# abiswas-odu/Disco

Hardware: AMD Instinct MI355X
Metric: overlaps/sec (BuildGraph stage), 150 bp reads (higher is better)
Workload: dtype u64; 1 GPU; 50000000 x 150 bp synthetic reads, 30x of 50 x 5000000 bp uniform-random contigs, both strands, error-free, min-overlap 40 (k=39), transitive reduction on, seed 42; reads=50000000, read_len=150, min_overlap=40, parallelism=1 GPU, e_pre=903537181, e_out=45314794, n_contained=4685156, cap_bind_sites=0, asymmetric_pairs=0, probes=5550000000, kmer_hits=2220071992

## Files before the change

disco_amd/build.py:

```python
from __future__ import annotations

import os
import shutil
import subprocess

HERE = os.path.dirname(os.path.abspath(__file__))
ROOT = os.path.dirname(HERE)
LIB = os.path.join(HERE, "libdisco_hip.so")
BUILDG = os.path.join(HERE, "bin", "buildG")

HIP_SOURCES = [os.path.join(HERE, "csrc", "disco_hip.hip")]
HIP_DEPS = HIP_SOURCES + [os.path.join(HERE, "csrc", f) for f in sorted(f for f in os.listdir(os.path.join(HERE, "csrc")) if f.endswith(".h"))] + [
    os.path.join(ROOT, "include", "disco_hip.h"), os.path.join(ROOT, "include", "disco_hip_test.h")]
HOST_SOURCES = [os.path.join(HERE, "host", f) for f in ("buildg_main.cpp", "fastx.cpp", "writer.cpp", "parsimple.cpp")]


def _hipcc() -> str:
    for cand in (shutil.which("hipcc"), "/opt/rocm/bin/hipcc"):
        if cand and os.path.exists(cand):
            return cand
    raise RuntimeError("hipcc not found: the HIP extension cannot be built")


def _stale(target: str, deps) -> bool:
    if not os.path.exists(target):
        return True
    t = os.path.getmtime(target)
    return any(os.path.exists(d) and os.path.getmtime(d) > t for d in deps)


def vgpr_spills(remarks: str) -> dict:
    out, name = {}, None
    for line in remarks.splitlines():
        if "Function Name:" in line:
            name = line.split("Function Name:")[1].split("[")[0].strip()
        elif "VGPRs Spill:" in line and name:
            n = int(line.split("VGPRs Spill:")[1].split("[")[0])
            if n:
                out[name] = n
    return out


def build_lib(force: bool = False, verbose: bool = False) -> str:
    if force or _stale(LIB, HIP_DEPS):
        tmp = LIB + ".tmp"
        cmd = [_hipcc(), "--offload-arch=gfx950", "-O3", "-std=c++17", "-fPIC", "-shared", "-pthread", "-Rpass-analysis=kernel-resource-usage",
               "-o", tmp] + HIP_SOURCES + ["-L/opt/rocm/lib", "-lrccl", "-lrocprofiler-sdk-roctx", "-Wl,-rpath,/opt/rocm/lib"]
        if verbose:
            print(" ".join(cmd))
        r = subprocess.run(cmd, stdout=subprocess.PIPE, stderr=subprocess.PIPE, text=True)
        if r.returncode != 0:
            raise RuntimeError("hipcc failed:\n" + "\n".join(l for l in r.stderr.splitlines() if "-Rpass-analysis" not in l)[-4000:])
        spills = vgpr_spills(r.stderr)
        if spills and not os.environ.get("DISCO_ALLOW_SPILLS"):
            os.unlink(tmp)
            raise RuntimeError(f"kernels spill vector registers (cross-lane reads would return garbage): {spills}")
        os.replace(tmp, LIB)
    return LIB


def build_host(force: bool = False, verbose: bool = False) -> str:
    srcs = [s for s in HOST_SOURCES if os.path.exists(s)]
    if not srcs:
        return ""
    deps = srcs + [os.path.join(HERE, "host", f) for f in os.listdir(os.path.join(HERE, "host")) if f.endswith(".h")] + [LIB]
    if force or _stale(BUILDG, deps):
        os.makedirs(os.path.dirname(BUILDG), exist_ok=True)
        cmd = ["g++", "-O2", "-std=c++17", "-fopenmp", "-Wall", "-I", os.path.join(ROOT, "include"), "-o", BUILDG] + srcs + [
            "-L", HERE, "-ldisco_hip", "-lz", "-Wl,-rpath,$ORIGIN/..", "-Wl,-rpath," + HERE]
        if verbose:
            print(" ".join(cmd))
        subprocess.check_call(cmd)
    dump = os.path.join(HERE, "bin", "fastx_dump")
    dsrc = [os.path.join(HERE, "host", "fastx_dump.cpp"), os.path.join(HERE, "host", "fastx.cpp")]
    if force or _stale(dump, dsrc + [os.path.join(HERE, "host", "fastx.h")]):
        cmd = ["g++", "-O2", "-std=c++17", "-fopenmp", "-Wall", "-o", dump] + dsrc + ["-lz"]
        if verbose:
            print(" ".join(cmd))
        subprocess.check_call(cmd)
    ps = os.path.join(HERE, "bin", "parsimplify")
    psrc = [os.path.join(HERE, "host", f) for f in ("parsimplify_main.cpp", "parsimple.cpp", "fastx.cpp", "writer.cpp")]
    if force or _stale(ps, psrc + [os.path.join(HERE, "host", f) for f in ("parsimple.h", "writer.h", "fastx.h")]):
        cmd = ["g++", "-O2", "-std=c++17", "-fopenmp", "-Wall", "-I", os.path.join(ROOT, "include"), "-o", ps] + psrc + ["-lz"]
        if verbose:
            print(" ".join(cmd))
        subprocess.check_call(cmd)
    gen = os.path.join(HERE, "bin", "readgen")
    gsrc = [os.path.join(HERE, "host", "readgen_main.cpp"), os.path.join(HERE, "csrc", "readgen.h")]
    if force or _stale(gen, gsrc):
        cmd = ["g++", "-O2", "-std=c++17", "-Wall", "-o", gen, gsrc[0]]
        if verbose:
            print(" ".join(cmd))
        subprocess.check_call(cmd)
    chk = os.path.join(HERE, "bin", "inflate_check")
    csrc = [os.path.join(HERE, "host", "inflate_check.cpp"), os.path.join(HERE, "csrc", "disco_inflate.h")]
    if force or _stale(chk, csrc):
        cmd = ["g++", "-O2", "-std=c++17", "-Wall", "-o", chk, csrc[0]]
        if verbose:
            print(" ".join(cmd))
        subprocess.check_call(cmd)
    return BUILDG


def build_all(force: bool = False, verbose: bool = False):
    build_lib(force, verbose)
    build_host(force, verbose)


if __name__ == "__main__":
    build_all(force=True, verbose=True)
```

disco_amd/buildgraph.py:

```python
from __future__ import annotations

import ctypes as C
import os

import numpy as np

_HERE = os.path.dirname(os.path.abspath(__file__))
_LIBPATH = os.environ.get("DISCO_LIB") or os.path.join(_HERE, "libdisco_hip.so")
_lib = None


class DiscoError(RuntimeError):
    pass


class Params(C.Structure):
    _fields_ = [("min_overlap", C.c_uint32), ("max_edges_per_kmer", C.c_uint32), ("flags", C.c_uint32), ("max_substitutions", C.c_uint32)]


class GenSpecABI(C.Structure):
    _fields_ = [("seed", C.c_uint64), ("n_reads", C.c_uint64), ("contig_len", C.c_uint64), ("n_contigs", C.c_uint32),
                ("len_min", C.c_uint32), ("len_max", C.c_uint32), ("skew", C.c_uint32)]


CONTAINED_DTYPE = np.dtype([("contained", "<u8"), ("super", "<u8"), ("orient", "<u4"), ("len2", "<u4"), ("len1", "<u4"),
                            ("start", "<u4"), ("j", "<u4"), ("type", "<u4")])
EDGE_DTYPE = np.dtype([("src", "<u8"), ("dst", "<u8"), ("orient", "<u4"), ("offset", "<u4"), ("len_src", "<u4"), ("len_dst", "<u4")])
COUNTER_NAMES = ("n_reads", "probes", "kmer_hits", "n_contained", "raw_hits", "e_pre", "e_out", "cap_bind_sites",
                 "asymmetric_pairs", "big_rows", "index_buckets", "hbm_bytes")


class Counters(C.Structure):
    _fields_ = [(n, C.c_uint64) for n in COUNTER_NAMES]


_P = C.c_void_p
ABI = [
    ("disco_abi_version", C.c_int, []),
    ("disco_create", C.c_int, [C.c_int, C.POINTER(Params), C.POINTER(_P)]),
    ("disco_destroy", None, [_P]),
    ("disco_last_error", C.c_char_p, [_P]),
    ("disco_set_stream", C.c_int, [_P, _P]),
    ("disco_synchronize", C.c_int, [_P]),
    ("disco_pack_ascii", C.c_int, [C.c_char_p, C.c_uint32, _P]),
    ("disco_host_alloc", _P, [C.c_size_t]),
    ("disco_host_free", None, [_P]),
    ("disco_upload_reads", C.c_int, [_P, _P, C.c_uint32, _P, C.c_uint64]),
    ("disco_adopt_reads", C.c_int, [_P, _P, C.c_uint32, _P, C.c_uint64]),
    ("disco_generate_reads", C.c_int, [_P, C.POINTER(GenSpecABI)]),
    ("disco_substitute_bases", C.c_int, [_P, C.c_uint64, C.c_uint32]),
    ("disco_download_reads", C.c_int, [_P, _P, _P]),
    ("disco_stride_words", C.c_uint32, [_P]),
    ("disco_num_reads", C.c_uint64, [_P]),
    ("disco_long_rows", C.c_uint64, [_P]),
    ("disco_upload_reads_ragged", C.c_int, [_P, _P, _P, C.c_uint64]),
    ("disco_set_query_range", C.c_int, [_P, C.c_uint64, C.c_uint64]),
    ("disco_build_index", C.c_int, [_P]),
    ("disco_probe", C.c_int, [_P]),
    ("disco_mark_contained", C.c_int, [_P, C.POINTER(C.c_uint64)]),
    ("disco_build_edges", C.c_int, [_P, C.POINTER(C.c_uint64)]),
    ("disco_select_edges", C.c_int, [_P]),
    ("disco_symmetrize", C.c_int, [_P, C.c_int, C.POINTER(C.c_uint64)]),
    ("disco_merge_extras", C.c_int, [_P]),
    ("disco_transitive_reduce", C.c_int, [_P, C.POINTER(C.c_uint64)]),
    ("disco_transitive_mark", C.c_int, [_P]),
    ("disco_emit_edges", C.c_int, [_P, C.POINTER(C.c_uint64)]),
    ("disco_run_graph", C.c_int, [_P]),
    ("disco_adjacency_size", C.c_int, [_P, C.POINTER(C.c_uint64)]),
    ("disco_export_adjacency", C.c_int, [_P, _P, _P]),
    ("disco_import_adjacency", C.c_int, [_P, _P, _P, C.c_uint64]),
    ("disco_fetch_contained", C.c_int64, [_P, _P, C.c_uint64]),
    ("disco_fetch_contained_grouped", C.c_int64, [_P, _P, C.c_uint64]),
    ("disco_fetch_edges", C.c_int64, [_P, _P, C.c_uint64]),
    ("disco_fetch_edge_substitutions", C.c_int64, [_P, _P, C.c_uint64]),
    ("disco_get_counters", C.c_int, [_P, C.POINTER(Counters)]),
    ("disco_phase_ms", C.c_int, [_P, C.POINTER(C.c_float), C.c_int]),
    ("disco_memcpy_d2d", C.c_int, [_P, _P, _P, C.c_uint64]),
    ("disco_fetch_edge_files", C.c_int64, [_P, C.c_uint32, _P, C.c_uint64]),
    ("disco_partition_edges", C.c_int64, [_P, _P, C.c_uint64, C.c_uint64, C.c_uint32, _P]),
    ("disco_format_edges", C.c_int64, [_P, C.c_uint32, _P, _P, _P]),
    ("disco_fetch_edge_text", C.c_int, [_P, _P, C.c_uint64]),
    ("disco_write_edge_text", C.c_int, [_P, _P, C.c_uint32, C.c_uint32]),
    ("disco_start_contained_rows", C.c_int, [_P, C.c_int]),
    ("disco_contract_chains", C.c_int, [_P, C.c_uint32, C.POINTER(C.c_uint64), C.POINTER(C.c_uint64)]),
    ("disco_contract_chains_of", C.c_int, [_P, _P, C.c_uint64, C.c_uint32, C.POINTER(C.c_uint64), C.POINTER(C.c_uint64)]),
    ("disco_fetch_chains", C.c_int, [_P, _P, _P, _P]),
    ("disco_set_query_order", C.c_int, [_P, _P]),
    ("disco_get_query_order", C.c_int, [_P, C.POINTER(_P)]),
    ("disco_probe_run_words", C.c_int, [_P]),
    ("disco_measure_hbm", C.c_int, [_P, C.c_uint64, C.c_int, C.POINTER(C.c_double)]),
    ("disco_measure_gather", C.c_int, [_P, C.c_uint64, C.c_int, C.POINTER(C.c_double)]),
    ("disco_comm_unique_id", C.c_int, [_P, C.c_size_t]),
    ("disco_comm_init", C.c_int, [_P, _P, C.c_int, C.c_int]),
    ("disco_comm_init_local", C.c_int, [C.POINTER(_P), C.c_int]),
    ("disco_comm_rank", C.c_int, [_P]),
    ("disco_comm_world", C.c_int, [_P]),
    ("disco_comm_kind", C.c_char_p, [_P]),
    ("disco_dist_range", C.c_int, [_P, C.c_uint64, C.POINTER(C.c_uint64), C.POINTER(C.c_uint64)]),
    ("disco_dist_upload_reads", C.c_int, [_P, _P, C.c_uint32, _P, C.c_uint64]),
    ("disco_dist_generate_reads", C.c_int, [_P, C.POINTER(GenSpecABI)]),
    ("disco_dist_run_graph", C.c_int, [_P, C.c_uint32]),
    ("disco_dist_get_info", C.c_int, [_P, _P]),
    ("disco_ingest_fasta", C.c_int, [_P, C.POINTER(C.c_char_p), C.c_int, C.c_uint32, _P, _P]),
    ("disco_ingest_fetch", C.c_int, [_P, _P, _P]),
    ("disco_inflate_bgzf", C.c_int64, [_P, _P, C.c_uint64, _P, C.c_uint64]),
]

ABI_VERSION = 2
FLAG_TWO_PASS_VERIFY = 1
XCHG = ("reads", "index_records", "index_shards", "contain", "row_requests", "row_data", "push", "adjacency", "twins", "queries", "hits", "keys", "reads_dealt", "contain_keys")
UNIQUE_ID_BYTES = 128
DIST_GATHER_READS = 1
DIST_KEEP_INDEX_PARTITIONED = 2


CHAIN_EDGE_DTYPE = np.dtype([("a", "<u8"), ("b", "<u8"), ("offset", "<u8"), ("orient", "<u4"), ("n_links", "<u4"), ("first_link", "<u8")])
CHAIN_LINK_DTYPE = np.dtype([("to", "<u4"), ("offset", "<u4"), ("orient", "<u4")])


class IngestFile(C.Structure):
    _fields_ = [("first_index", C.c_uint64), ("last_index", C.c_uint64), ("good", C.c_uint64), ("bad", C.c_uint64)]


class IngestInfo(C.Structure):
    _fields_ = [("n_reads", C.c_uint64), ("total_records", C.c_uint64), ("too_long", C.c_uint64), ("stride_words", C.c_uint32), ("shortest", C.c_uint32),
                ("longest", C.c_uint32), ("read_s", C.c_float), ("device_s", C.c_float)]


class DistInfo(C.Structure):
    _fields_ = [("world", C.c_uint32), ("rank", C.c_uint32), ("n_reads", C.c_uint64), ("own_lo", C.c_uint64), ("own_hi", C.c_uint64),
                ("n_contained", C.c_uint64), ("e_pre", C.c_uint64), ("e_out", C.c_uint64), ("e_out_local", C.c_uint64),
                ("n_contained_local", C.c_uint64), ("cap_bind_sites", C.c_uint64), ("asymmetric_pairs", C.c_uint64),
                ("dropped_hits", C.c_uint64), ("probes", C.c_uint64), ("kmer_hits", C.c_uint64), ("regime", C.c_uint32),
                ("tr_rounds", C.c_uint32), ("tr_deferred", C.c_uint64), ("bytes_sent", C.c_uint64 * len(XCHG)),
                ("ms", C.c_float * len(XCHG)), ("ms_total", C.c_float), ("kernel_ms", C.c_float), ("comm_ops", C.c_uint32),
                ("host_syncs", C.c_uint32), ("device_allocs", C.c_uint32), ("device_frees", C.c_uint32), ("arena_bytes", C.c_uint64),
                ("arena_peak", C.c_uint64), ("hbm_peak", C.c_uint64), ("own_reads", C.c_uint64), ("placement", C.c_uint32), ("reserved_", C.c_uint32)]

PHASES = ("index", "probe_kernel", "verify", "contain", "select", "csr", "twin", "trmark", "emit", "order")


def lib_path() -> str:
    return _LIBPATH


def load():
    global _lib
    if _lib is None:
        if not os.path.exists(_LIBPATH):
            raise DiscoError(f"{_LIBPATH} is missing: build it with `python -m disco_amd.build` (hipcc, gfx950). "
                             "There is no CPU fallback.")
        L = C.CDLL(_LIBPATH)
        L.disco_abi_version.restype = C.c_int
        if L.disco_abi_version() != ABI_VERSION:
            raise DiscoError(f"{_LIBPATH} speaks ABI version {L.disco_abi_version()}, this mirror was written against {ABI_VERSION}: rebuild "
                             "(`python -m disco_amd.build`)")
        for name, res, args in ABI:
            fn = getattr(L, name)
            fn.restype = res
            fn.argtypes = args
        _lib = L
    return _lib


class BuildGraph:

    def __init__(self, min_overlap: int = 40, device: int = 0, max_edges_per_kmer: int = 4, flags: int = 0, max_substitutions: int = 0):
        self.L = load()
        self.min_overlap = min_overlap
        self._h = _P()
        p = Params(min_overlap, max_edges_per_kmer, flags, max_substitutions)
        rc = self.L.disco_create(device, C.byref(p), C.byref(self._h))
        if rc != 0:
            raise DiscoError(f"disco_create failed ({rc}): {self.L.disco_last_error(None).decode()}")

    def _chk(self, rc):
        if rc < 0:
            raise DiscoError(f"libdisco_hip error {rc}: {self.L.disco_last_error(self._h).decode()}")
        return rc

    def close(self):
        if self._h:
            self.L.disco_destroy(self._h)
            self._h = _P()

    def __del__(self):
        try:
            self.close()
        except Exception:
            pass

    def __enter__(self):
        return self

    def __exit__(self, *a):
        self.close()

    def set_stream(self, stream_ptr: int | None):
        self._chk(self.L.disco_set_stream(self._h, _P(stream_ptr) if stream_ptr else None))

    def synchronize(self):
        self._chk(self.L.disco_synchronize(self._h))

    def upload_reads(self, packed: np.ndarray, lens: np.ndarray):
        packed = np.ascontiguousarray(packed, dtype=np.uint64)
        lens = np.ascontiguousarray(lens, dtype=np.uint16)
        assert packed.ndim == 2 and packed.shape[0] == lens.shape[0]
        self._keep = (packed, lens)
        self._chk(self.L.disco_upload_reads(self._h, packed.ctypes.data, packed.shape[1], lens.ctypes.data, packed.shape[0]))

    def upload_reads_ragged(self, words: np.ndarray, lens: np.ndarray):
        words = np.ascontiguousarray(words, dtype=np.uint64)
        lens = np.ascontiguousarray(lens, dtype=np.uint16)
        assert words.ndim == 1 and len(words) == int(((lens.astype(np.int64) + 31) // 32).sum())
        self._chk(self.L.disco_upload_reads_ragged(self._h, words.ctypes.data, lens.ctypes.data, len(lens)))

    def upload_ascii(self, reads, ragged: bool = False):
        n = len(reads)
        lens = np.fromiter((len(r) for r in reads), dtype=np.uint16, count=n)
        if ragged:
            off = np.zeros(n + 1, dtype=np.int64)
            np.cumsum((lens.astype(np.int64) + 31) // 32, out=off[1:])
            words = np.zeros(max(int(off[-1]), 1), dtype=np.uint64)
            for i, r in enumerate(reads):
                b = r.encode()
                if self.L.disco_pack_ascii(b, len(b), words[off[i]:].ctypes.data) != 0:
                    raise DiscoError(f"read {i} contains a non-ACGT base")
            return self.upload_reads_ragged(words[:int(off[-1])], lens)
        stride = int((int(lens.max()) + 31) // 32) if n else 1
        packed = np.zeros((n, stride), dtype=np.uint64)
        for i, r in enumerate(reads):
            b = r.encode()
            if self.L.disco_pack_ascii(b, len(b), packed[i].ctypes.data) != 0:
                raise DiscoError(f"read {i} contains a non-ACGT base")
        self.upload_reads(packed, lens)

    def adopt_reads(self, d_packed_ptr: int, stride_words: int, d_len_ptr: int, n: int):
        self._chk(self.L.disco_adopt_reads(self._h, _P(d_packed_ptr), stride_words, _P(d_len_ptr), n))

    def generate_reads(self, spec):
        s = GenSpecABI(spec.seed, spec.n_reads, spec.contig_len, spec.n_contigs, spec.len_min, spec.len_max, int(spec.skew_word if hasattr(spec, "skew_word") else getattr(spec, "skew", 0)))
        self._chk(self.L.disco_generate_reads(self._h, C.byref(s)))

    def substitute_bases(self, seed: int, rate_ppm: int):
        self._chk(self.L.disco_substitute_bases(self._h, seed, rate_ppm))

    def download_reads(self):
        n, s = self.num_reads, self.stride_words
        packed = np.zeros((n, s), dtype=np.uint64)
        lens = np.zeros(n, dtype=np.uint16)
        self._chk(self.L.disco_download_reads(self._h, packed.ctypes.data, lens.ctypes.data))
        return packed, lens

    @property
    def num_reads(self) -> int:
        return int(self.L.disco_num_reads(self._h))

    @property
    def stride_words(self) -> int:
        return int(self.L.disco_stride_words(self._h))

    @property
    def long_rows(self) -> int:
        return int(self.L.disco_long_rows(self._h))

    def set_query_range(self, lo: int, hi: int):
        self._chk(self.L.disco_set_query_range(self._h, lo, hi))

    def build_index(self):
        self._chk(self.L.disco_build_index(self._h))

    def probe(self):
        self._chk(self.L.disco_probe(self._h))

    def mark_contained(self) -> int:
        n = C.c_uint64()
        self._chk(self.L.disco_mark_contained(self._h, C.byref(n)))
        return n.value

    def build_edges(self) -> int:
        n = C.c_uint64()
        self._chk(self.L.disco_build_edges(self._h, C.byref(n)))
        return n.value

    def select_edges(self):
        self._chk(self.L.disco_select_edges(self._h))

    def symmetrize(self, full: bool) -> int:
        n = C.c_uint64()
        self._chk(self.L.disco_symmetrize(self._h, 1 if full else 0, C.byref(n)))
        return n.value

    def merge_extras(self):
        self._chk(self.L.disco_merge_extras(self._h))

    def transitive_reduce(self) -> int:
        n = C.c_uint64()
        self._chk(self.L.disco_transitive_reduce(self._h, C.byref(n)))
        return n.value

    def transitive_mark(self):
        self._chk(self.L.disco_transitive_mark(self._h))

    def emit_edges(self) -> int:
        n = C.c_uint64()
        self._chk(self.L.disco_emit_edges(self._h, C.byref(n)))
        return n.value

    def run_graph(self):
        self._chk(self.L.disco_run_graph(self._h))

    def adjacency_size(self) -> int:
        n = C.c_uint64()
        self._chk(self.L.disco_adjacency_size(self._h, C.byref(n)))
        return n.value

    def export_adjacency(self, d_deg_ptr: int, d_entries_ptr: int):
        self._chk(self.L.disco_export_adjacency(self._h, _P(d_deg_ptr), _P(d_entries_ptr)))

    def import_adjacency(self, d_deg_all_ptr: int, d_entries_all_ptr: int, n_entries: int):
        self._chk(self.L.disco_import_adjacency(self._h, _P(d_deg_all_ptr), _P(d_entries_all_ptr), n_entries))

    def fetch_contained(self) -> np.ndarray:
        n = self._chk(self.L.disco_fetch_contained(self._h, None, 0))
        out = np.zeros(n, dtype=CONTAINED_DTYPE)
        if n:
            self._chk(self.L.disco_fetch_contained(self._h, out.ctypes.data, n))
        return out

    def fetch_contained_grouped(self):
        n = self._chk(self.L.disco_fetch_contained_grouped(self._h, None, 0))
        out = np.zeros(n, dtype=CONTAINED_DTYPE)
        if n:
            rc = self.L.disco_fetch_contained_grouped(self._h, out.ctypes.data, n)
            if rc == -6:
                return None
            self._chk(rc)
        return out

    def fetch_edges(self) -> np.ndarray:
        n = self._chk(self.L.disco_fetch_edges(self._h, None, 0))
        out = np.zeros(n, dtype=EDGE_DTYPE)
        if n:
            self._chk(self.L.disco_fetch_edges(self._h, out.ctypes.data, n))
        return out

    def format_edges(self, n_files: int = 1, edge_file=None, file_index=None):
        off = np.zeros(n_files + 1, dtype=np.uint64)
        ef = None if edge_file is None else np.ascontiguousarray(edge_file, dtype=np.uint16)
        fi = None if file_index is None else np.ascontiguousarray(file_index, dtype=np.uint64)
        nb = self._chk(self.L.disco_format_edges(self._h, n_files, None if ef is None else ef.ctypes.data, None if fi is None else fi.ctypes.data, off.ctypes.data))
        buf = np.empty(max(nb, 1), dtype=np.uint8)
        self._chk(self.L.disco_fetch_edge_text(self._h, buf.ctypes.data, nb))
        return buf[:nb].tobytes(), off

    def write_edge_text(self, fds, threads: int = 8):
        arr = (C.c_int * len(fds))(*fds)
        self._chk(self.L.disco_write_edge_text(self._h, arr, len(fds), threads))

    def start_contained_rows(self, grouped: bool = False):
        self._chk(self.L.disco_start_contained_rows(self._h, 1 if grouped else 0))

    def contract_chains(self, min_overlap_simplify: int = 0, edges=None):
        nc, nl = C.c_uint64(), C.c_uint64()
        if edges is None:
            self._chk(self.L.disco_contract_chains(self._h, min_overlap_simplify, C.byref(nc), C.byref(nl)))
            ne = int(self.L.disco_fetch_edges(self._h, None, 0))
        else:
            edges = np.ascontiguousarray(edges, dtype=EDGE_DTYPE)
            self._chk(self.L.disco_contract_chains_of(self._h, edges.ctypes.data, len(edges), min_overlap_simplify, C.byref(nc), C.byref(nl)))
            ne = len(edges)
        comp = np.zeros(nc.value, dtype=CHAIN_EDGE_DTYPE)
        links = np.zeros(nl.value, dtype=CHAIN_LINK_DTYPE)
        absorbed = np.zeros(ne, dtype=np.uint8)
        self._chk(self.L.disco_fetch_chains(self._h, comp.ctypes.data if len(comp) else None, links.ctypes.data if len(links) else None,
                                            absorbed.ctypes.data if ne else None))
        return comp, links, absorbed

    def fetch_edge_substitutions(self) -> np.ndarray:
        n = self._chk(self.L.disco_fetch_edge_substitutions(self._h, None, 0))
        out = np.zeros(n, dtype=np.uint16)
        if n:
            self._chk(self.L.disco_fetch_edge_substitutions(self._h, out.ctypes.data, n))
        return out

    def phase_ms(self) -> dict:
        a = (C.c_float * len(PHASES))()
        self._chk(self.L.disco_phase_ms(self._h, a, len(PHASES)))
        return {n: float(a[i]) for i, n in enumerate(PHASES)}

    def fetch_edge_files(self, n_files: int):
        n = int(self.L.disco_fetch_edges(self._h, None, 0))
        out = np.zeros(max(n, 1), dtype=np.uint16)
        self._chk(self.L.disco_fetch_edge_files(self._h, n_files, out.ctypes.data, n))
        return out[:n]

    def partition_edges(self, edges: np.ndarray, n_nodes: int, n_files: int):
        edges = np.ascontiguousarray(edges, dtype=EDGE_DTYPE)
        out = np.zeros(max(len(edges), 1), dtype=np.uint16)
        self._chk(self.L.disco_partition_edges(self._h, edges.ctypes.data, len(edges), n_nodes, n_files, out.ctypes.data))
        return out[:len(edges)]

    def get_query_order(self) -> int:
        out = _P()
        self._chk(self.L.disco_get_query_order(self._h, C.byref(out)))
        return out.value or 0

    def set_query_order(self, d_order_ptr: int):
        self._chk(self.L.disco_set_query_order(self._h, _P(d_order_ptr)))

    def probe_run_words(self) -> int:
        return int(self.L.disco_probe_run_words(self._h))

    def measure_hbm(self, nbytes: int = 4 << 30, reps: int = 5) -> float:
        out = C.c_double(0.0)
        self._chk(self.L.disco_measure_hbm(self._h, nbytes, reps, C.byref(out)))
        return out.value

    def measure_gather(self, nbytes: int = 3 << 30, reps: int = 3) -> float:
        out = C.c_double(0.0)
        self._chk(self.L.disco_measure_gather(self._h, nbytes, reps, C.byref(out)))
        return out.value

    def memcpy_d2d(self, dst_ptr: int, src_ptr: int, nbytes: int):
        self._chk(self.L.disco_memcpy_d2d(self._h, _P(dst_ptr), _P(src_ptr), nbytes))

    @staticmethod
    def comm_unique_id() -> bytes:
        buf = C.create_string_buffer(UNIQUE_ID_BYTES)
        rc = load().disco_comm_unique_id(buf, UNIQUE_ID_BYTES)
        if rc != 0:
            raise DiscoError(f"disco_comm_unique_id failed ({rc})")
        return buf.raw

    def comm_init(self, unique_id: bytes, world: int, rank: int):
        self._chk(self.L.disco_comm_init(self._h, C.c_char_p(unique_id), world, rank))

    @staticmethod
    def comm_init_local(graphs):
        arr = (_P * len(graphs))(*[g._h for g in graphs])
        rc = load().disco_comm_init_local(arr, len(graphs))
        if rc != 0:
            raise DiscoError(f"disco_comm_init_local failed ({rc})")

    @property
    def rank(self) -> int:
        return int(self.L.disco_comm_rank(self._h))

    @property
    def world(self) -> int:
        return int(self.L.disco_comm_world(self._h))

    @property
    def transport(self) -> str:
        return self.L.disco_comm_kind(self._h).decode()

    def dist_range(self, n_total: int):
        lo, hi = C.c_uint64(), C.c_uint64()
        self._chk(self.L.disco_dist_range(self._h, n_total, C.byref(lo), C.byref(hi)))
        return lo.value, hi.value

    def dist_upload_reads(self, packed_own: np.ndarray, lens_own: np.ndarray, n_total: int, stride_words: int | None = None):
        packed_own = np.ascontiguousarray(packed_own, dtype=np.uint64)
        lens_own = np.ascontiguousarray(lens_own, dtype=np.uint16)
        self._keep = (packed_own, lens_own)
        stride = int(stride_words if stride_words is not None else packed_own.shape[1])
        self._chk(self.L.disco_dist_upload_reads(self._h, packed_own.ctypes.data, stride, lens_own.ctypes.data, n_total))

    def dist_upload_ascii(self, reads):
        n = len(reads)
        lo, hi = self.dist_range(n)
        stride = int((max((len(r) for r in reads), default=1) + 31) // 32)
        packed = np.zeros((hi - lo, stride), dtype=np.uint64)
        lens = np.fromiter((len(r) for r in reads[lo:hi]), dtype=np.uint16, count=hi - lo)
        for i, r in enumerate(reads[lo:hi]):
            b = r.encode()
            if self.L.disco_pack_ascii(b, len(b), packed[i].ctypes.data) != 0:
                raise DiscoError(f"read {lo + i} contains a non-ACGT base")
        self.dist_upload_reads(packed, lens, n, stride)

    def dist_generate_reads(self, spec):
        s = GenSpecABI(spec.seed, spec.n_reads, spec.contig_len, spec.n_contigs, spec.len_min, spec.len_max, int(spec.skew_word if hasattr(spec, "skew_word") else getattr(spec, "skew", 0)))
        self._chk(self.L.disco_dist_generate_reads(self._h, C.byref(s)))

    def ingest_fasta(self, paths, threads: int = 16):
        arr = (C.c_char_p * len(paths))(*[os.fsencode(p) for p in paths])
        info, files = IngestInfo(), (IngestFile * len(paths))()
        rc = self.L.disco_ingest_fasta(self._h, arr, len(paths), threads, C.byref(info), files)
        if rc == -6:
            return None
        self._chk(rc)
        return ({n: getattr(info, n) for n, _ in IngestInfo._fields_}, [{n: getattr(f, n) for n, _ in IngestFile._fields_} for f in files])

    def inflate_bgzf(self, data: bytes):
        data = bytes(data)
        n = self.L.disco_inflate_bgzf(self._h, data, len(data), None, 0)
        if n == -6:
            return None
        out = C.create_string_buffer(max(self._chk(n), 1))
        n = self.L.disco_inflate_bgzf(self._h, data, len(data), out, n)
        if n == -6:
            return None
        return out.raw[:self._chk(n)]

    def last_error(self) -> str:
        return self.L.disco_last_error(self._h).decode()

    def ingest_fetch(self):
        n = self.num_reads
        ln, fi = np.zeros(n, dtype=np.uint16), np.zeros(n, dtype=np.uint64)
        self._chk(self.L.disco_ingest_fetch(self._h, ln.ctypes.data, fi.ctypes.data))
        return ln, fi

    def dist_run_graph(self, gather_reads: bool = True, partitioned_index: bool = False):
        self._chk(self.L.disco_dist_run_graph(self._h, (DIST_GATHER_READS if gather_reads else 0) | (DIST_KEEP_INDEX_PARTITIONED if partitioned_index else 0)))

    def dist_info(self) -> dict:
        d = DistInfo()
        self._chk(self.L.disco_dist_get_info(self._h, C.byref(d)))
        out = {n: getattr(d, n) for n, _ in DistInfo._fields_ if n not in ("bytes_sent", "ms")}
        out["bytes_sent"] = {x: int(d.bytes_sent[i]) for i, x in enumerate(XCHG)}
        out["ms"] = {x: float(d.ms[i]) for i, x in enumerate(XCHG)}
        return out

    def host_to_host_pass(self, passes: int = 2) -> dict:
        import time

        n, s = self.num_reads, self.stride_words
        p = self.L.disco_host_alloc(max(n * s * 8, 8))
        if not p:
            raise DiscoError("disco_host_alloc failed")
        q = None
        try:
            lens = np.zeros(n, dtype=np.uint16)
            self._chk(self.L.disco_download_reads(self._h, p, lens.ctypes.data))
            w = max(1, (int(lens.max()) + 31) // 32) if n else 1
            src, sw = p, s
            if w < s:
                q = self.L.disco_host_alloc(max(n * w * 8, 8))
                if not q:
                    raise DiscoError("disco_host_alloc failed")
                full = np.ctypeslib.as_array(C.cast(p, C.POINTER(C.c_uint64)), shape=(n, s))
                np.ctypeslib.as_array(C.cast(q, C.POINTER(C.c_uint64)), shape=(n, w))[:] = full[:, :w]
                src, sw = q, w
            rows = edges = None
            out, first = {}, None
            for ip in range(max(1, passes)):
                t0 = time.perf_counter()
                self._chk(self.L.disco_upload_reads(self._h, src, sw, lens.ctypes.data, n))
                t1 = time.perf_counter()
                self.run_graph()
                self.synchronize()
                t2 = time.perf_counter()
                nc = self._chk(self.L.disco_fetch_contained(self._h, None, 0))
                ne = self._chk(self.L.disco_fetch_edges(self._h, None, 0))
                if rows is None or len(rows) < nc or len(edges) < ne:
                    rows = np.zeros(max(nc, 1), dtype=CONTAINED_DTYPE)
                    edges = np.zeros(max(ne, 1), dtype=EDGE_DTYPE)
                t3 = time.perf_counter()
                if nc:
                    self._chk(self.L.disco_fetch_contained(self._h, rows.ctypes.data, nc))
                t4 = time.perf_counter()
                if ne:
                    self._chk(self.L.disco_fetch_edges(self._h, edges.ctypes.data, ne))
                t5 = time.perf_counter()
# ... 17 lines not shown
```

disco_amd/csrc/disco_hip.hip:

```cpp
#include <hip/hip_runtime.h>
#include <rocprofiler-sdk-roctx/roctx.h>

#include <algorithm>
#include <atomic>
#include <chrono>
#include <cstdarg>
#include <cstdio>
#include <cstdlib>
#include <cstring>
#include <fcntl.h>
#include <sys/mman.h>
#include <sys/stat.h>
#include <unistd.h>
#include <string>
#include <memory>
#include <thread>
#include <map>
#include <mutex>
#include <vector>

#include "../../include/disco_hip.h"
#include "../../include/disco_hip_test.h"
#include "disco_kernels.h"
#include "disco_dist.h"

#define DROP_LIST_CAP (1u << 20)
#include "disco_chains.h"
#include "disco_text.h"
#include "disco_ingest.h"
#include "disco_bgzf.h"
#include "read_filter_tables.h"
#include "disco_comm.h"

static_assert(sizeof(disco_genspec) == sizeof(disco_genspec_abi), "genspec ABI mismatch");

static thread_local std::string g_create_error;

using HClock = std::chrono::steady_clock;
static float ms_since(HClock::time_point t0) { return std::chrono::duration<float, std::milli>(HClock::now() - t0).count(); }

#define DISCO_PH_INDEX2 DISCO_PH_COUNT
#define DISCO_PH_SLOTS (DISCO_PH_COUNT + 1)

struct RoctxRange {
    explicit RoctxRange(const char *name) { (void)roctxRangePushA(name); }
    ~RoctxRange() { (void)roctxRangePop(); }
    RoctxRange(const RoctxRange &) = delete;
    RoctxRange &operator=(const RoctxRange &) = delete;
};
#define DISCO_TRACE(name) RoctxRange roctx_range_(name)

template <typename F>
static void parallel_for(u64 n, F f)
{
    unsigned nt = std::thread::hardware_concurrency();
    if (const char *e = getenv("DISCO_HOST_THREADS")) nt = (unsigned)atoi(e);
    nt = std::max(1u, std::min(nt, 16u));
    if (n < (1u << 16) || nt == 1) {
        f((u64)0, n);
        return;
    }
    std::vector<std::thread> th;
    for (unsigned t = 0; t < nt; t++) th.emplace_back([=]() { f(n * t / nt, n * (t + 1) / nt); });
    for (auto &x : th) x.join();
}


struct PassCounters {
    u32 dev_allocs = 0, dev_frees = 0, host_syncs = 0, comm_ops = 0;
};
static thread_local PassCounters tl_pass;
static inline hipError_t counted_stream_sync(hipStream_t s)
{
    tl_pass.host_syncs++;
    return hipStreamSynchronize(s);
}
static inline hipError_t counted_event_sync(hipEvent_t e)
{
    tl_pass.host_syncs++;
    return hipEventSynchronize(e);
}
#define hipStreamSynchronize(s) counted_stream_sync(s)
#define hipEventSynchronize(e) counted_event_sync(e)

struct DevArena {
    char *base = nullptr;
    size_t size = 0, used = 0, peak = 0;
    std::map<size_t, size_t> free_at;
    bool owns(const void *p) const { return base && (const char *)p >= base && (const char *)p < base + size; }
    void *alloc(size_t bytes)
    {
        bytes = (bytes + 255) & ~(size_t)255;
        for (auto it = free_at.begin(); it != free_at.end(); ++it)
            if (it->second >= bytes) {
                const size_t off = it->first, len = it->second;
                free_at.erase(it);
                if (len > bytes) free_at[off + bytes] = len - bytes;
                live[off] = bytes;
                used += bytes;
                peak = std::max(peak, used);
                return base + off;
            }
        return nullptr;
    }
    void release(void *p)
    {
        const size_t off = (size_t)((char *)p - base);
        auto lv = live.find(off);
        if (lv == live.end()) return;
        size_t start = off, end = off + lv->second;
        used -= lv->second;
        live.erase(lv);
        auto nx = free_at.lower_bound(off);
        if (nx != free_at.end() && nx->first == end) {
            end += nx->second;
            nx = free_at.erase(nx);
        }
        if (nx != free_at.begin()) {
            auto pv = std::prev(nx);
            if (pv->first + pv->second == start) {
                start = pv->first;
                free_at.erase(pv);
            }
        }
        free_at[start] = end - start;
    }
    std::map<size_t, size_t> live;
};

template <typename T>
struct DevBuf {
    T *p = nullptr;
    u64 cap = 0;
    operator T *() const { return p; }
};

struct disco_ctx {
    int device = 0;
    disco_params prm{};
    DevArena arena;
    int k = 0;
    hipStream_t own_stream = nullptr;
    hipStream_t stream = nullptr;
    int n_cu = 256;
    std::string err;
    size_t hbm_bytes = 0, hbm_peak = 0;

    u64 n = 0;
    int S = 0;
    u64 *d_reads = nullptr;
    u16 *d_len = nullptr;
    DevBuf<u64> reads_own;
    DevBuf<u16> len_own;
    bool reads_owned = false;
    std::vector<uint16_t> h_len;
    bool h_len_ok = false;
    std::mutex h_len_mu;
    u64 q_lo = 0, q_hi = 0;
    bool two_class = false;
    bool dist_two_class = false;
    u64 job_n_long = 0;
    u32 job_short_max = 0;
    int S_ext = 0;
    u64 n_long = 0;
    DevBuf<u64> d_full;
    DevBuf<u32> d_ovf, d_long_ids;
    u32 max_len_all = 0;
    int tailb = 0;
    DevBuf<u32> d_lpos, d_n_list;
    DevBuf<uint2> d_linfo;
    DevBuf<ulonglong2> d_lmeta;

    u64 T = 0;
    int bshift = 0;
    DevBuf<u32> d_bkt;
    DevBuf<u64> d_ent;
    DevBuf<ulonglong2> d_rec;
    bool binned_index = false;
    DevBuf<ulonglong2> d_rec2;
    DevBuf<u32> d_binx;

    DevBuf<u64> d_tile;
    u64 *d_total = nullptr;

    u64 *d_ctr = nullptr;
    u64 *d_wq = nullptr;
    u64 h_ctr[CTR_COUNT] = {0};

    DevBuf<u64> d_best;
    DevBuf<u64> d_hits;
    u64 hits_used = 0;
    u64 *d_bump = nullptr;
    DevBuf<u64> d_row_start;
    DevBuf<u32> d_row_cnt;
    DevBuf<u64> d_big_list;
    DevBuf<u32> d_big_cnt;
    u32 *d_n_big = nullptr;
    DevBuf<u32> d_runs;
    u64 runs_lo = 0, runs_n = 0;
    int runs_lpr = 0;
    DevBuf<u64> d_slow_list;
    u32 *d_n_slow = nullptr;
    u64 big_rows = 0, slow_rows = 0;
    const u64 *d_order = nullptr;
    const u64 *d_order_used = nullptr;
    bool order_external = false;
    DevBuf<u32> d_ocnt, d_okey, d_oslot;
    DevBuf<u64> d_order_own;
    bool order_counted = false;
    bool es_big_counted = false, tr_big_counted = false;
    bool contained_count_pending = false;
    bool order_ready = false;
    hipStream_t aux_stream = nullptr;
    hipEvent_t ev_crows = nullptr;
    DevBuf<u32> d_cpos, d_crow_id;
    DevBuf<u64> d_crow_key;
    DevBuf<u64> d_tile2;
    u64 *d_total2 = nullptr;
    void *h_crows = nullptr;
    DevBuf<u32> d_crow_len;
    u64 crows_hcap = 0, crows_n = 0;
    bool crows_pending = false;
    bool crows_in_ring = false;
    DevBuf<u32> d_cgrp_cur, d_cgrp_id;
    DevBuf<u64> d_cgrp_key, d_cgrp_big;
    u64 h_cgrp_big = 0;
    bool cgrp_pending = false;
    DevBuf<u32> d_fetch_src;
    DevBuf<u64> d_fetch_ent;
    DevBuf<u32> d_rec_of_read;
    std::vector<u64> ingest_id_base, ingest_rec_base;
    u64 ingest_n = 0;
    void *h_ring = nullptr;
    std::vector<u64> text_off;
    DevBuf<u8> d_ingest;
    std::thread hits_prealloc;
    DevBuf<u64> prealloc;
    size_t ring_half = 0;
    hipEvent_t ev_ring[2] = {nullptr, nullptr};
    hipStream_t copy_stream = nullptr;
    hipEvent_t ev_copied[3] = {nullptr, nullptr, nullptr}, ev_unpacked[3] = {nullptr, nullptr, nullptr};
    bool index_counted = false;
    u64 order_counted_lo = 0, order_counted_hi = 0;
    int order_counted_bits = 0;
    DevBuf<u32> d_asked;
    u64 order_q_lo = 0, order_q_hi = 0;
    DevBuf<ulonglong2> d_meta_ord;
    u64 dropped_local = 0;
    ProbeRare h_probe_rare;
    DevBuf<ProbeRare> d_probe_rare;
    u32 max_len = 0, min_len = 0;
    bool two_pass_last = false;
    bool contained_done = false;

    DevBuf<u8> d_contained;
    DevBuf<u64> d_cbits;
    DevBuf<u64> d_dropbits;
    DevBuf<u64> d_drop_node, d_drop_key;
    u64 n_drop_items = 0;
    u64 drop_lo = 0, drop_hi = 0;
    u64 n_contained = 0;

    DevBuf<u64> d_adj_ref;
    u64 *d_adj = nullptr;
    DevBuf<u64> d_adj_own;
    DevBuf<u64> d_adj_spare;
    DevBuf<u64> d_start_tmp;
    u64 adj_total = 0;
    bool flags_pending = false;
    bool adj_imported = false;
    u64 adj_span = 0;
    bool half_complete = false;
    DevBuf<u32> d_extra_cnt;
    DevBuf<u64> d_extra_node, d_extra_key;
    u32 *d_n_extra = nullptr;
    u32 n_extra = 0;
    u64 asym_local = 0;
    u64 dropped = 0;

    DevBuf<u64> d_half;
    DevBuf<u32> d_hcnt;
    bool use_half = false;
    DevBuf<u64> d_wide;
    DevBuf<u32> d_n_wide;
    u32 n_wide = 0;
    DevBuf<u8> d_out_valid;
    DevBuf<u64> d_out_pos;
    u64 *h_stage = nullptr;
    hipEvent_t ev_stage[2] = {nullptr, nullptr};
    DevBuf<ChainEdgeOut> d_ch_comp;
    DevBuf<ChainLinkOut> d_ch_links;
    DevBuf<u8> d_ch_dead;
    u64 ch_comp_n = 0, ch_links_n = 0, ch_edges_n = 0;
    bool ch_ready = false;
    DevBuf<char> d_text;
    u64 text_bytes = 0;
    DevBuf<u64> d_out_src, d_out_ent;
    u64 out_used = 0;
    u64 n_out = 0;

    hipEvent_t ev0[DISCO_PH_SLOTS] = {nullptr}, ev1[DISCO_PH_SLOTS] = {nullptr};
    bool ev_pending[DISCO_PH_SLOTS] = {false};
    float ph_ms[DISCO_PH_SLOTS] = {0};

    int phase = 0;

    DiscoComm *comm = nullptr;
    DiscoComm *comm_bulk = nullptr;
    hipStream_t bulk_stream = nullptr;
    hipEvent_t ev_bulk = nullptr;
    bool wait_bulk_before_verify = false;
    u64 per = 0;
    u64 n_alloc = 0;
    bool part_index = false;
    u64 part_blo = 0, part_bhi = 0, part_nrec = 0;
    DevBuf<u64> d_pq_start;
    bool dist_reads = false;
    bool dist_active = false;
    DevBuf<u64> d_route;
    DevBuf<ulonglong2> d_x16a, d_x16b;
    DevBuf<u32> d_req_flat, d_req_s, d_req_r;
    DevBuf<u32> d_rdeg_s, d_rdeg_r, d_rdata_s;
    DevBuf<u64> d_rpos;
    DevBuf<u32> d_nadj32_own;
    u64 nadj_used = 0;
    DevBuf<u32> d_deg_tmp;
    DevBuf<u64> d_list_n;
    DevBuf<u64> d_dense;
    ulonglong2 *d_push_r = nullptr;
    u64 n_push_r = 0;
    bool loci = false;
    bool runs_by_pos = false;
    DevBuf<u8> d_otab;
    DevBuf<u32> d_own_ids;
    u64 n_own = 0;
    u64 home_lo = 0, home_hi = 0;
    u64 home_probes = 0;
    DevBuf<u64> d_cb_all;
    hipEvent_t ev_keys = nullptr, ev_keys_go = nullptr;
    bool keys_pending = false;
    disco_dist_info dinfo{};
    bool time_exchanges = false;
    unsigned dist_passes = 0;
};

static int fail(disco_ctx *c, int code, const char *fmt, ...)
{
    char buf[512];
    va_list ap;
    va_start(ap, fmt);
    vsnprintf(buf, sizeof buf, fmt, ap);
    va_end(ap);
    if (c) c->err = buf;
    else g_create_error = buf;
    return code;
}

#define HIPCHK(c, call)                                                                                          \
    do {                                                                                                         \
        hipError_t e_ = (call);                                                                                  \
        if (e_ != hipSuccess) return fail((c), e_ == hipErrorOutOfMemory ? DISCO_E_NOMEM : DISCO_E_HIP, "%s failed: %s (%s:%d)", #call, hipGetErrorString(e_), __FILE__, __LINE__); \
    } while (0)
// ... 231 lines not shown

template <typename InT, typename OutT>
static int scan_exclusive_on(disco_ctx *c, hipStream_t st, DevBuf<u64> &tile, u64 *total, const InT *in, u64 n, OutT *out, bool write_total, u64 *total_host)
{
    u64 nt = (n + SCAN_TILE - 1) / SCAN_TILE;
    if (nt == 0) nt = 1;
    CHK(ensure(c, tile, nt));
    hipLaunchKernelGGL((scan_tile_sums_kernel<InT>), dim3((unsigned)nt), dim3(SCAN_BLOCK), 0, st, in, n, tile.p);
    hipLaunchKernelGGL(scan_sums_kernel, dim3(1), dim3(1024), 0, st, tile.p, nt, total);
    hipLaunchKernelGGL((scan_apply_kernel<InT, OutT>), dim3((unsigned)nt), dim3(SCAN_BLOCK), 0, st, in, n, tile.p, out);
    if (write_total) hipLaunchKernelGGL((scan_write_total_kernel<OutT>), dim3(1), dim3(1), 0, st, total, out + n);
    HIPCHK(c, hipGetLastError());
    if (total_host) {
        HIPCHK(c, hipMemcpyAsync(total_host, total, sizeof(u64), hipMemcpyDeviceToHost, st));
        HIPCHK(c, hipStreamSynchronize(st));
    }
    return DISCO_OK;
}

template <typename InT, typename OutT>
static int scan_exclusive(disco_ctx *c, const InT *in, u64 n, OutT *out, bool write_total, u64 *total_host)
{
    return scan_exclusive_on<InT, OutT>(c, c->stream, c->d_tile, c->d_total, in, n, out, write_total, total_host);
}

static void free_graph_state(disco_ctx *c)
{
    if (c->keys_pending) {
        c->keys_pending = false;
        if (c->ev_keys) (void)hipEventSynchronize(c->ev_keys);
    }
    release(c, c->d_bkt);
    release(c, c->d_ent);
    release(c, c->d_rec);
    release(c, c->d_rec2);
    release(c, c->d_binx);
    release(c, c->d_best);
    release(c, c->d_hits);
    release(c, c->d_row_start);
    release(c, c->d_row_cnt);
    release(c, c->d_big_list);
    release(c, c->d_big_cnt);
    release(c, c->d_slow_list);
    release(c, c->d_runs);
    c->runs_n = 0;
    c->runs_lpr = 0;
    release(c, c->d_contained);
    release(c, c->d_cbits);
    release(c, c->d_dropbits);
    release(c, c->d_drop_node);
    release(c, c->d_drop_key);
    release(c, c->d_adj_ref);
    release(c, c->d_adj_own);
    release(c, c->d_adj_spare);
    release(c, c->d_start_tmp);
    release(c, c->d_ocnt);
    release(c, c->d_okey);
    release(c, c->d_meta_ord);
    release(c, c->d_asked);
    release(c, c->d_oslot);
    release(c, c->d_order_own);
    c->d_order_used = nullptr;
    c->d_adj = nullptr;
    release(c, c->d_extra_cnt);
    release(c, c->d_extra_node);
    release(c, c->d_extra_key);
    release(c, c->d_half);
    release(c, c->d_hcnt);
    release(c, c->d_wide);
    release(c, c->d_n_wide);
    c->adj_total = 0;
    release(c, c->d_out_valid);
    release(c, c->d_ch_comp);
    release(c, c->d_ch_links);
    release(c, c->d_ch_dead);
    release(c, c->d_text);
    c->text_bytes = 0;
    c->ch_ready = false;
    release(c, c->d_out_pos);
    release(c, c->d_out_src);
    release(c, c->d_out_ent);
    c->n_out = c->out_used = 0;
    c->flags_pending = false;
    c->adj_imported = false;
    c->T = 0;
    release(c, c->d_x16a);
    release(c, c->d_x16b);
    release(c, c->d_req_flat);
    release(c, c->d_req_s);
    release(c, c->d_req_r);
    release(c, c->d_rdeg_s);
    release(c, c->d_rdeg_r);
    release(c, c->d_rdata_s);
    release(c, c->d_rpos);
    release(c, c->d_nadj32_own);
    release(c, c->d_deg_tmp);
    release(c, c->d_dense);
    release(c, c->d_pq_start);
    c->nadj_used = 0;
    c->d_push_r = nullptr;
    c->n_push_r = 0;
    release(c, c->d_cb_all);
    release(c, c->d_otab);
    release(c, c->d_own_ids);
    c->n_own = 0;
    c->loci = c->runs_by_pos = false;
}

static void free_long_class(disco_ctx *c)
{
    release(c, c->d_full);
    release(c, c->d_ovf);
    release(c, c->d_long_ids);
    release(c, c->d_lpos);
    release(c, c->d_lmeta);
    release(c, c->d_linfo);
    release(c, c->d_n_list);
    c->two_class = false;
    c->n_long = 0;
    c->S_ext = 0;
    c->tailb = 0;
}

static void free_reads(disco_ctx *c)
{
    release(c, c->reads_own);
    release(c, c->len_own);
    free_long_class(c);
    c->d_reads = nullptr;
    c->d_len = nullptr;
    c->reads_owned = false;
    c->h_len.clear();
    c->n = 0;
}

static int alloc_reads(disco_ctx *c, u64 words, u64 n_len)
{
    CHK(ensure(c, c->reads_own, words));
    c->d_reads = c->reads_own;
    CHK(ensure(c, c->len_own, n_len));
    c->d_len = c->len_own;
    return DISCO_OK;
}

static u32 extra_cap(const disco_ctx *c) { return (u32)std::min<u64>(std::min(c->d_extra_node.cap, c->d_extra_key.cap), 0xFFFFFFFFull); }

static int grow_big_lists(disco_ctx *c, u64 need) { return ensure_group(c, need, need, c->d_big_list, c->d_big_cnt); }

static bool own_order_wanted(const disco_ctx *c, u64 nq, int *bits)
{
    const u64 order_min = getenv("DISCO_ORDER_MIN_READS") ? (u64)atoll(getenv("DISCO_ORDER_MIN_READS")) : 4096;
    int b = 16;
    while (b < 27 && (1ull << b) < nq) ++b;
    *bits = b;
    return !c->order_external && !getenv("DISCO_NO_ORDER") && nq >= order_min && nq > 0;
}

struct IndexCountPlan {
    u64 lo = 0, hi = 0;
    int lpr = 0, nf = 0;
    u32 *ocnt = nullptr, *oslot = nullptr;
    u32 oshift = 0;
    const u64 *list = nullptr;
};

static bool runs_nf_built(int nf, int m) { return (nf == 7 || nf == 12 || nf == 17 || nf == 22 || nf == 27) && m == RUNS_M; }

static int runs_lpr_for(const disco_ctx *c, int nf, u32 max_len, u64 nloc)
{
    int lpr = 0;
    const int m = view(c).m;
    const bool nf_built = runs_nf_built(nf, m);
    const bool nf_generic = nf >= 2 && nf <= 64 && m > 16 && m <= 31 && !getenv("DISCO_NO_GENERIC_RUNS");
    if ((nf_built || nf_generic) && max_len > (u32)c->k && !getenv("DISCO_NO_RUNS")) {
        const u32 maxwin = max_len - (u32)c->k;
        const u32 expect = 2u * maxwin / (u32)(nf + 1);
        lpr = maxwin <= 256 ? (maxwin <= 128 && expect <= 20 ? 16 : (expect <= 44 ? 32 : 0)) : 0;
        const double max_gb = getenv("DISCO_RUNS_MAX_GB") ? atof(getenv("DISCO_RUNS_MAX_GB")) : 16.0;
        if ((double)nloc * lpr * 4.0 > max_gb * 1e9) lpr = 0;
    }
    return lpr;
}

static bool two_class_ok(const disco_ctx *c, int S, u64 n, u64 n_long, u32 short_max, bool will_own = false)
{
    if (((c->comm || c->dist_reads) && !c->dist_two_class) || !(c->reads_owned || will_own) || c->prm.max_substitutions || getenv("DISCO_NO_TWO_CLASS")) return false;
    if (S <= VERIFY_SW || n_long == 0 || n_long * (u64)env_int("DISCO_TWO_CLASS_ONE_IN", 5) > n || n + n_long >= (1ull << 31)) return false;
    return runs_lpr_for(c, c->k - view(c).m + 1, short_max, n) != 0;
}

static int two_class_alloc(disco_ctx *c, u64 n_long, int Sx, u32 short_max);

static int index_count_plan(disco_ctx *c, const DiscoView &v, u64 lo, u64 hi, IndexCountPlan *pl, const u64 *list = nullptr)
{
    const u64 nloc = hi - lo;
    *pl = IndexCountPlan();
    pl->lo = lo;
    pl->hi = hi;
    pl->list = list;
    if (!list) c->order_counted = c->order_ready = false;
    int obits = 0;
    if (!list && lo == c->q_lo && hi == c->q_hi && own_order_wanted(c, nloc, &obits) && !getenv("DISCO_NO_ORDER_FUSE")) {
        const u64 order_buckets = 1ull << obits;
        CHK(ensure(c, c->d_ocnt, order_buckets + 1));
        CHK(ensure(c, c->d_oslot, nloc));
        HIPCHK(c, hipMemsetAsync(c->d_ocnt, 0, (order_buckets + 1) * sizeof(u32), c->stream));
        pl->ocnt = c->d_ocnt;
        pl->oslot = c->d_oslot;
        pl->oshift = 32u - (u32)obits;
        c->order_counted = true;
        c->order_counted_lo = lo;
        c->order_counted_hi = hi;
        c->order_counted_bits = obits;
    }
    c->runs_lpr = 0;
    c->runs_n = 0;
    c->runs_by_pos = false;
    const int nf = v.k - v.m + 1;
    const int lpr = c->S == VERIFY_SW ? runs_lpr_for(c, nf, c->max_len, nloc) : 0;
    if (lpr && nloc) {
        CHK(ensure(c, c->d_runs, nloc * (u64)lpr));
        c->runs_lpr = lpr;
        c->runs_lo = lo;
        c->runs_n = nloc;
        c->runs_by_pos = list != nullptr;
        pl->lpr = lpr;
        pl->nf = nf;
    }
    return DISCO_OK;
}

typedef void (*IndexRunsFn)(DiscoView, u32 *, ulonglong2 *, u32 *, u64, u64, u32 *, u32 *, u32 *, u32, const u64 *);
typedef void (*IndexCountFn)(DiscoView, u32 *, ulonglong2 *, u32 *, u64, u64, u32 *, u32 *, u32, const u64 *);
struct IndexCountKernel {
    IndexRunsFn runs = nullptr;
    IndexCountFn plain = nullptr;
};
template <bool COUNT, int NF, int NFMAX, bool LONGK>
static IndexCountKernel index_runs_pick(int lpr)
{
    IndexCountKernel k;
    k.runs = lpr == 16 ? index_runs_kernel<COUNT, NF, 1, NFMAX, LONGK> : index_runs_kernel<COUNT, NF, 2, NFMAX, LONGK>;
    return k;
}
template <bool COUNT>
static IndexCountKernel index_count_pick(int nf, int m, int lpr, bool longk, bool long_class)
{
    if (long_class || !lpr) {
        IndexCountKernel k;
        if (long_class) k.plain = longk ? index_count_kernel<COUNT, true, true> : index_count_kernel<COUNT, false, true>;
        else k.plain = longk ? index_count_kernel<COUNT, true> : index_count_kernel<COUNT>;
        return k;
    }
    if (runs_nf_built(nf, m)) switch (nf) {
        case 7: return index_runs_pick<COUNT, 7, 7, false>(lpr);
        case 12: return index_runs_pick<COUNT, 12, 12, false>(lpr);
        case 17: return index_runs_pick<COUNT, 17, 17, false>(lpr);
        case 22: return index_runs_pick<COUNT, 22, 22, false>(lpr);
        default: return index_runs_pick<COUNT, 27, 27, false>(lpr);
        }
    if (longk) return nf <= 48 ? index_runs_pick<COUNT, 0, 48, true>(lpr) : index_runs_pick<COUNT, 0, 64, true>(lpr);
    if (nf <= 8) return index_runs_pick<COUNT, 0, 8, false>(lpr);
    if (nf <= 12) return index_runs_pick<COUNT, 0, 12, false>(lpr);
    if (nf <= 16) return index_runs_pick<COUNT, 0, 16, false>(lpr);
    if (nf <= 24) return index_runs_pick<COUNT, 0, 24, false>(lpr);
    if (nf <= 32) return index_runs_pick<COUNT, 0, 32, false>(lpr);
    if (nf <= 48) return index_runs_pick<COUNT, 0, 48, false>(lpr);
    return index_runs_pick<COUNT, 0, 64, false>(lpr);
}
static IndexCountKernel index_count_pick(bool count, int nf, int m, int lpr, bool longk, bool long_class)
{
    return count ? index_count_pick<true>(nf, m, lpr, longk, long_class) : index_count_pick<false>(nf, m, lpr, longk, long_class);
}

static int index_count_chunk(disco_ctx *c, const DiscoView &v, const IndexCountPlan &pl, bool count, ulonglong2 *rec_base, u64 a, u64 b)
{
    if (b <= a) return DISCO_OK;
    const dim3 grid((unsigned)((b - a + 255) / 256));
    ulonglong2 *rec = rec_base + 2 * (a - pl.lo);
    u32 *oslot = pl.oslot ? pl.oslot + (a - pl.lo) : nullptr;
    u32 *okey = pl.list ? nullptr : c->d_okey.p;
    const IndexCountKernel k = index_count_pick(count, pl.nf, v.m, pl.lpr, c->k > 64, false);
    if (k.runs) hipLaunchKernelGGL(k.runs, grid, dim3(256), 0, c->stream, v, c->d_bkt, rec, okey, a, b, c->d_runs + (a - pl.lo) * (u64)pl.lpr, pl.ocnt, oslot, pl.oshift, pl.list);
    else hipLaunchKernelGGL(k.plain, grid, dim3(256), 0, c->stream, v, c->d_bkt, rec, okey, a, b, pl.ocnt, oslot, pl.oshift, pl.list);
    HIPCHK(c, hipGetLastError());
    return DISCO_OK;
}

static int index_count_long(disco_ctx *c, const DiscoView &v, const IndexCountPlan &pl, bool count, ulonglong2 *rec, u32 *oslot, u64 x_lo, u64 x_hi)
{
    const dim3 g((unsigned)((x_hi - x_lo + 255) / 256));
    hipLaunchKernelGGL(index_count_pick(count, 0, v.m, 0, c->k > 64, true).plain, g, dim3(256), 0, c->stream, v, c->d_bkt, rec, c->d_okey, x_lo, x_hi, pl.ocnt, oslot, pl.oshift,
                       (const u64 *)nullptr);
    HIPCHK(c, hipGetLastError());
    return DISCO_OK;
}

static bool binned_index_wanted(disco_ctx *c, int logT)
{
    if (getenv("DISCO_NO_BINNED_INDEX") || 2 * c->n >= 0xFFFF0000ull) return false;
    if (logT > BINX_SPAN_BITS && ensure(c, c->d_rec2, 2 * c->n) != DISCO_OK) {
        (void)hipGetLastError();
        c->err.clear();
        return false;
    }
    return true;
}

static int size_bucket_table(disco_ctx *c)
{
    u64 T = 1024;
    int logT = 10;
    double tscale = 2.0;
    if (const char *e = getenv("DISCO_BUCKET_SCALE")) tscale = atof(e);
    while ((double)T < tscale * (double)c->n && logT < 32) {
        T <<= 1;
        logT++;
    }
    c->T = T;
    c->bshift = 64 - logT;
    return logT;
}

static int index_begin(disco_ctx *c)
{
    const int logT = size_bucket_table(c);
    const u64 T = c->T;
    CHK(ensure(c, c->d_bkt, T + 1));
    CHK(ensure(c, c->d_ent, 2 * c->n));
    CHK(ensure(c, c->d_rec, 2 * c->n));
    CHK(ensure(c, c->d_okey, c->n));
    c->adj_imported = false;
    c->binned_index = binned_index_wanted(c, logT);
    if (!c->binned_index) HIPCHK(c, hipMemsetAsync(c->d_bkt, 0, (T + 1) * sizeof(u32), c->stream));
    return DISCO_OK;
}

struct BinxPlan {
    int span = 0, levels = 0, bits[3] = {0, 0, 0};
};
static BinxPlan binx_plan(int logT)
{
    BinxPlan b;
    b.span = std::min(logT, BINX_SPAN_BITS);
    const int prefix = logT - b.span;
    b.levels = (prefix + BINX_MAX_BITS - 1) / BINX_MAX_BITS;
    for (int l = 0; l < b.levels; l++) b.bits[l] = prefix / b.levels + (l < prefix % b.levels ? 1 : 0);
    return b;
}

static int binned_build_index(disco_ctx *c)
{
    const int logT = 64 - c->bshift;
    const BinxPlan bp = binx_plan(logT);
    const u32 total = (u32)(2 * c->n);
    const u32 n_part = 1u << (logT - bp.span);
    const u32 tiles = (total + BINX_TILE - 1u) / BINX_TILE;
    u64 hist_len = 1;
    for (int l = 0, done = 0; l < bp.levels; done += bp.bits[l], l++) hist_len = std::max<u64>(hist_len, ((u64)tiles + (1ull << done)) * (1ull << bp.bits[l]) + 1);
    const u64 tab = ((u64)n_part + 1 + 63) & ~63ull;
    CHK(ensure(c, c->d_binx, 4 * tab + hist_len));
    u32 *seg[2] = {c->d_binx.p, c->d_binx.p + tab}, *tb[2] = {c->d_binx.p + 2 * tab, c->d_binx.p + 3 * tab}, *hist = c->d_binx.p + 4 * tab;
    if (getenv("DISCO_VERBOSE"))
        fprintf(stderr, "[disco] binned index build: 2^%d buckets, %u partitions of 2^%d, %d level(s) of %d / %d / %d bits\n", logT, n_part, bp.span, bp.levels, bp.bits[0], bp.bits[1], bp.bits[2]);
    ulonglong2 *src = c->d_rec, *dst = c->d_rec2;
    u32 pseg = 1, pnb = 1;
    int cur = 0, done = 0;
    for (int l = 0; l < bp.levels; l++) {
        const u32 nseg = 1u << done, nb = 1u << bp.bits[l], shift = (u32)(logT - done - bp.bits[l]);
        const u32 grid = tiles + nseg;
        const u64 hlen = (u64)grid * nb + 1;
        hipLaunchKernelGGL(binx_segs_kernel, dim3(1), dim3(1024), 0, c->stream, l ? (const u32 *)hist : (const u32 *)nullptr, (const u32 *)tb[cur ^ 1], pseg, pnb, total, seg[cur], tb[cur]);
        HIPCHK(c, hipMemsetAsync(hist, 0, hlen * sizeof(u32), c->stream));
        hipLaunchKernelGGL(binx_hist_kernel, dim3(grid), dim3(BINX_BLOCK), 0, c->stream, (const ulonglong2 *)src, (const u32 *)seg[cur], (const u32 *)tb[cur], nseg, shift, nb, hist);
        CHK((scan_exclusive<u32, u32>(c, hist, hlen, hist, false, nullptr)));
        hipLaunchKernelGGL(binx_scatter_kernel, dim3(grid), dim3(BINX_BLOCK), 0, c->stream, (const ulonglong2 *)src, dst, (const u32 *)seg[cur], (const u32 *)tb[cur], nseg, shift, nb,
                           (const u32 *)hist);
        HIPCHK(c, hipGetLastError());
        std::swap(src, dst);
        pseg = nseg;
        pnb = nb;
        done += bp.bits[l];
        cur ^= 1;
    }
    hipLaunchKernelGGL(binx_segs_kernel, dim3(1), dim3(1024), 0, c->stream, bp.levels ? (const u32 *)hist : (const u32 *)nullptr, (const u32 *)tb[cur ^ 1], pseg, pnb, total, seg[cur],
                       (u32 *)nullptr);
    hipLaunchKernelGGL(binx_build_kernel, dim3(n_part), dim3(BINX_BUILD_BLOCK), 0, c->stream, (const ulonglong2 *)src, (const u32 *)seg[cur], (u32)bp.span, total, c->T, c->d_bkt.p, c->d_ent.p);
    HIPCHK(c, hipGetLastError());
    return DISCO_OK;
}

static int start_contained_rows(disco_ctx *c, bool grouped)
{
    const u64 nc = c->n_contained;
    if (c->crows_pending && c->crows_n == nc && (!grouped || c->cgrp_pending)) return DISCO_OK;
    const bool have_rows = c->crows_pending && c->crows_n == nc;
    if (!have_rows) c->crows_pending = c->cgrp_pending = false;
    const u64 max_rows = getenv("DISCO_EAGER_ROWS_MAX") ? (u64)atoll(getenv("DISCO_EAGER_ROWS_MAX")) : (16ull << 20);
    if (c->comm || nc == 0 || nc > max_rows || c->n >= (1ull << 31)) return DISCO_OK;
    if (!c->aux_stream) {
        HIPCHK(c, hipStreamCreateWithFlags(&c->aux_stream, hipStreamNonBlocking));
        HIPCHK(c, hipEventCreateWithFlags(&c->ev_crows, hipEventDisableTiming));
        HIPCHK(c, hipMalloc((void **)&c->d_total2, sizeof(u64)));
    }
    CHK(ensure(c, c->d_cpos, c->n + 1));
    CHK(ensure_group(c, nc, nc + nc / 4 + 1024, c->d_crow_id, c->d_crow_key, c->d_crow_len));
    if (nc > c->crows_hcap && c->h_ring && !c->crows_in_ring && (u64)c->ring_half * 2 >= (nc + 1024) * 32) {
        if (c->h_crows) (void)hipHostFree(c->h_crows);
        c->h_crows = c->h_ring;
        c->crows_hcap = (u64)c->ring_half * 2 / 32;
        c->crows_in_ring = true;
    }
    if (nc > c->crows_hcap) {
        if (c->h_crows && !c->crows_in_ring) (void)hipHostFree(c->h_crows);
        c->crows_in_ring = false;
        c->h_crows = nullptr;
        c->crows_hcap = 0;
        const u64 want = nc + nc / 4 + 1024;
        if (hipHostMalloc(&c->h_crows, want * 32) != hipSuccess) {
            c->h_crows = nullptr;
            (void)hipGetLastError();
            return DISCO_OK;
        }
        c->crows_hcap = want;
    }
    if (!have_rows) {
    CHK((scan_exclusive_on<u8, u32>(c, c->aux_stream, c->d_tile2, c->d_total2, c->d_contained, c->n, c->d_cpos, false, nullptr)));
    hipLaunchKernelGGL(contain_rows32_kernel, dim3(flat_grid(c, c->n)), dim3(256), 0, c->aux_stream, c->d_best, c->d_contained, c->d_cpos, c->n, c->d_crow_id, c->d_crow_key);
    HIPCHK(c, hipGetLastError());
    u64 *hkey = (u64 *)c->h_crows;
    u32 *hid = (u32 *)(hkey + c->crows_hcap), *hln = hid + c->crows_hcap;
    hipLaunchKernelGGL(crow_lens_kernel, dim3(flat_grid(c, nc)), dim3(256), 0, c->aux_stream, (const u32 *)c->d_crow_id, (const u64 *)c->d_crow_key, nc, (const u16 *)c->d_len, c->d_crow_len);
    HIPCHK(c, hipGetLastError());
    HIPCHK(c, hipMemcpyAsync(hkey, c->d_crow_key, nc * 8, hipMemcpyDeviceToHost, c->aux_stream));
    HIPCHK(c, hipMemcpyAsync(hid, c->d_crow_id, nc * 4, hipMemcpyDeviceToHost, c->aux_stream));
    HIPCHK(c, hipMemcpyAsync(hln, c->d_crow_len, nc * 4, hipMemcpyDeviceToHost, c->aux_stream));
    HIPCHK(c, hipEventRecord(c->ev_crows, c->aux_stream));
    c->crows_n = nc;
    c->crows_pending = true;
    }
    if (grouped && !c->cgrp_pending) {
        CHK(ensure(c, c->d_cgrp_cur, c->n + 1));
        CHK(ensure_group(c, nc, nc + nc / 4 + 1024, c->d_cgrp_id, c->d_cgrp_key));
        CHK(ensure(c, c->d_cgrp_big, 1));
        HIPCHK(c, hipMemsetAsync(c->d_cpos, 0, (c->n + 1) * sizeof(u32), c->aux_stream));
        HIPCHK(c, hipMemsetAsync(c->d_cgrp_big, 0, sizeof(u64), c->aux_stream));
        hipLaunchKernelGGL(crow_count_kernel, dim3(flat_grid(c, nc)), dim3(256), 0, c->aux_stream, (const u64 *)c->d_crow_key, nc, c->d_cpos);
        CHK((scan_exclusive_on<u32, u32>(c, c->aux_stream, c->d_tile2, c->d_total2, c->d_cpos, c->n + 1, c->d_cgrp_cur, false, nullptr)));
        hipLaunchKernelGGL(crow_place_kernel, dim3(flat_grid(c, nc)), dim3(256), 0, c->aux_stream, (const u32 *)c->d_crow_id, (const u64 *)c->d_crow_key, nc, c->d_cgrp_cur, c->d_cgrp_id,
                           c->d_cgrp_key);
        hipLaunchKernelGGL(crow_sort_groups_kernel, dim3(flat_grid(c, nc)), dim3(256), 0, c->aux_stream, c->d_cgrp_id, c->d_cgrp_key, nc, c->d_cgrp_big);
        HIPCHK(c, hipGetLastError());
        u64 *gkey = (u64 *)((char *)c->h_crows + c->crows_hcap * 16);
        u32 *gid = (u32 *)(gkey + c->crows_hcap), *gln = gid + c->crows_hcap;
        hipLaunchKernelGGL(crow_lens_kernel, dim3(flat_grid(c, nc)), dim3(256), 0, c->aux_stream, (const u32 *)c->d_cgrp_id, (const u64 *)c->d_cgrp_key, nc, (const u16 *)c->d_len, c->d_crow_len);
        HIPCHK(c, hipMemcpyAsync(gkey, c->d_cgrp_key, nc * 8, hipMemcpyDeviceToHost, c->aux_stream));
        HIPCHK(c, hipMemcpyAsync(gid, c->d_cgrp_id, nc * 4, hipMemcpyDeviceToHost, c->aux_stream));
        HIPCHK(c, hipMemcpyAsync(gln, c->d_crow_len, nc * 4, hipMemcpyDeviceToHost, c->aux_stream));
        HIPCHK(c, hipMemcpyAsync(&c->h_cgrp_big, c->d_cgrp_big, sizeof(u64), hipMemcpyDeviceToHost, c->aux_stream));
        c->cgrp_pending = true;
    }
    return DISCO_OK;
}

static int settle_contained_rows(disco_ctx *c)
{
    if (c->crows_pending) HIPCHK(c, hipStreamSynchronize(c->aux_stream));
    c->crows_pending = false;
    c->cgrp_pending = false;
    return DISCO_OK;
}

static int ring_back_from_rows(disco_ctx *c)
{
    if (!c->crows_in_ring) return DISCO_OK;
    if (c->crows_pending && c->aux_stream) HIPCHK(c, hipStreamSynchronize(c->aux_stream));
    c->crows_pending = c->cgrp_pending = false;
    c->h_crows = nullptr;
    c->crows_hcap = 0;
    c->crows_in_ring = false;
    return DISCO_OK;
}

static void settle_hits_prealloc(disco_ctx *c)
{
    if (!c->hits_prealloc.joinable()) return;
    c->hits_prealloc.join();
    if (c->prealloc) {
        if (c->prealloc.cap > c->d_hits.cap) {
            release(c, c->d_hits);
            adopt(c, c->d_hits, c->prealloc);
        } else
            (void)hipFree(c->prealloc.p);
        c->prealloc = DevBuf<u64>();
    }
}


typedef void (*ProbeFn)(ProbeArgs);
typedef void (*ProbeRunsFn)(ProbeArgs, const u32 *, u64);
struct ProbeKernel {
    ProbeRunsFn runs = nullptr;
    ProbeFn plain = nullptr;
};
template <int PMODE>
static ProbeFn probe_mode_pick(bool ldsrow, bool row17, bool longk, bool long_class)
{
    if constexpr (PMODE != 0) {
        if (long_class) return longk ? probe_kernel<PMODE, false, false, true, true> : row17 ? probe_kernel<PMODE, false, true, false, true> : probe_kernel<PMODE, false, false, false, true>;
    }
    if constexpr (PMODE != 2) {
        if (!ldsrow) return longk ? probe_kernel<PMODE, false, false, true> : row17 ? probe_kernel<PMODE, false, true> : probe_kernel<PMODE, false, false>;
    }
    return longk ? probe_kernel<PMODE, true, false, true> : row17 ? probe_kernel<PMODE, true, true> : probe_kernel<PMODE, true, false>;
}
static ProbeKernel probe_pick(const disco_ctx *c, int mode, bool use_runs)
{
    const bool ldsrow = c->S <= PROBE_ACAP;
    const bool row17 = c->k - view(c).m == 16 && !getenv("DISCO_NO_ROW17");
    const bool longk = c->k > 64;
    const bool long_class = c->two_class && c->S_ext > PROBE_ACAP;
    ProbeKernel k;
    if (mode == 0 && use_runs) k.runs = c->runs_lpr == 16 ? probe_runs_kernel<16> : probe_runs_kernel<32>;
    else if (mode == 0) k.plain = probe_mode_pick<0>(ldsrow, row17, longk, long_class);
    else if (mode == 1) k.plain = probe_mode_pick<1>(ldsrow, row17, longk, long_class);
    else k.plain = probe_mode_pick<2>(ldsrow, row17, longk, long_class);
    return k;
}

typedef void (*VerifyFn)(VerifyArgs);
template <bool INEXACT>
static VerifyFn verify_rows_pick(int S, bool short_rows)
{
    if (S == VERIFY_SW) return short_rows ? verify_kernel<5, 0, INEXACT> : verify_kernel<8, 0, INEXACT>;
    return S == 16 ? verify_kernel<16, 0, INEXACT> : S == 24 ? verify_kernel<24, 0, INEXACT> : S == 32 ? verify_kernel<32, 0, INEXACT> : verify_kernel<0, 0, INEXACT>;
}
template <int MODE>
static VerifyFn verify_pass_pick(bool flat, bool short_rows)
{
    if (flat) return short_rows ? verify_flat_kernel<5, MODE> : verify_flat_kernel<8, MODE>;
// ... 1132 lines not shown
    if (s->len_min == 0 || s->len_max < s->len_min || longest > 32767 || s->n_contigs == 0 || s->contig_len < longest)
        return fail(c, DISCO_E_ARG, "disco_generate_reads: bad spec");
    HIPCHK(c, hipSetDevice(c->device));
    uint32_t stride = (((longest + 31) / 32) + 7u) & ~7u;
    bool kept = false;
    CHK(set_reads_common(c, s->n_reads, stride, &kept));
    if (!kept) CHK(alloc_reads(c, c->n * (u64)stride, c->n));
    c->reads_owned = true;
    disco_genspec g;
    memcpy(&g, s, sizeof g);
    if (c->n) hipLaunchKernelGGL(generate_reads_kernel, dim3(flat_grid(c, c->n * stride)), dim3(256), 0, c->stream, g, c->d_reads, c->d_len, (int)stride, (u64)0, c->n);
    HIPCHK(c, hipGetLastError());
    return validate_reads(c);
}

int disco_substitute_bases(disco_ctx *c, uint64_t seed, uint32_t rate_ppm)
{
    if (!c) return DISCO_E_ARG;
    if (c->phase != 1) return fail(c, DISCO_E_STATE, "disco_substitute_bases: call after the reads are set and before disco_build_index");
    if (rate_ppm > 1000000) return fail(c, DISCO_E_ARG, "disco_substitute_bases: rate above 10^6 ppm");
    if (c->two_class)
        return fail(c, DISCO_E_UNSUPPORTED, "disco_substitute_bases: the table has two classes of rows (reads of more than 256 bases next to short ones); substitute "
                                            "into generated reads, or set DISCO_NO_TWO_CLASS=1");
    HIPCHK(c, hipSetDevice(c->device));
    const u64 lo = c->comm ? c->q_lo : 0, hi = c->comm ? c->q_hi : c->n;
    if (hi > lo && rate_ppm)
        hipLaunchKernelGGL(substitute_bases_kernel, dim3(flat_grid(c, (hi - lo) * (u64)c->S)), dim3(256), 0, c->stream, (u64)seed, rate_ppm, c->d_reads, c->d_len, c->S, lo, hi);
    c->index_counted = c->order_counted = c->order_ready = false;
    HIPCHK(c, hipGetLastError());
    return DISCO_OK;
}

int disco_download_reads(disco_ctx *c, uint64_t *packed, uint16_t *len)
{
    if (!c || c->phase < 1) return c ? fail(c, DISCO_E_STATE, "no reads") : DISCO_E_ARG;
    HIPCHK(c, hipSetDevice(c->device));
    DevBuf<u64> joined;
    if (packed && c->n && c->two_class) {
        CHK(ensure(c, joined, c->n * (u64)c->S_ext));
        hipLaunchKernelGGL(class_join_kernel, dim3(flat_grid(c, c->n * (u64)c->S_ext)), dim3(256), 0, c->stream, (const u64 *)c->d_reads, (const u64 *)c->d_full, c->S_ext,
                           (const u16 *)c->d_len, (const u32 *)c->d_ovf, c->n, joined);
        (void)hipMemcpyAsync(packed, joined, c->n * (u64)c->S_ext * 8, hipMemcpyDeviceToHost, c->stream);
    } else if (packed && c->n)
        HIPCHK(c, hipMemcpyAsync(packed, c->d_reads, c->n * (u64)c->S * 8, hipMemcpyDeviceToHost, c->stream));
    if (len && c->n) (void)hipMemcpyAsync(len, c->d_len, c->n * 2, hipMemcpyDeviceToHost, c->stream);
    const hipError_t e = hipStreamSynchronize(c->stream);
    release(c, joined);
    if (e != hipSuccess) return fail(c, DISCO_E_HIP, "disco_download_reads: %s", hipGetErrorString(e));
    return DISCO_OK;
}

uint32_t disco_stride_words(const disco_ctx *c) { return c ? (uint32_t)(c->two_class ? c->S_ext : c->S) : 0; }
uint64_t disco_num_reads(const disco_ctx *c) { return c ? c->n : 0; }
uint64_t disco_long_rows(const disco_ctx *c) { return c && c->two_class ? c->n_long : 0; }

int disco_set_query_range(disco_ctx *c, uint64_t lo, uint64_t hi)
{
    if (!c) return DISCO_E_ARG;
    if (c->phase < 1 || c->phase > 2) return fail(c, DISCO_E_STATE, "disco_set_query_range: call after the reads are set and before disco_probe");
    if (lo > hi || hi > c->n) return fail(c, DISCO_E_ARG, "query range [%llu,%llu) outside [0,%llu)", (unsigned long long)lo, (unsigned long long)hi, (unsigned long long)c->n);
    c->q_lo = lo;
    c->q_hi = hi;
    return DISCO_OK;
}

static int two_class_alloc(disco_ctx *c, u64 n_long, int Sx, u32 short_max)
{
    c->n_long = n_long;
    c->S_ext = Sx;
    int rc = DISCO_OK;
    rc = ensure(c, c->d_ovf, c->n_alloc);
    if (rc == DISCO_OK) rc = ensure(c, c->d_full, n_long * (u64)Sx);
    if (rc == DISCO_OK) rc = ensure(c, c->d_long_ids, n_long);
    if (rc == DISCO_OK) rc = ensure(c, c->d_lpos, n_long);
    if (rc == DISCO_OK) rc = ensure(c, c->d_lmeta, n_long);
    if (rc == DISCO_OK) rc = ensure(c, c->d_linfo, n_long);
    if (rc == DISCO_OK) rc = ensure(c, c->d_n_list, 1);
    if (rc != DISCO_OK) {
        free_long_class(c);
        return rc;
    }
    c->S = VERIFY_SW;
    c->tailb = short_max <= 160 ? 160 : 256;
    c->two_class = true;
    if (getenv("DISCO_VERBOSE"))
        fprintf(stderr, "[disco] two classes of rows: %llu of %llu reads are longer than 256 bases, the others up to %u: 64-byte rows + %d-word rows for those\n",
                (unsigned long long)n_long, (unsigned long long)c->n, short_max, Sx);
    return DISCO_OK;
}

static int two_class_convert(disco_ctx *c)
{
    if (c->two_class || !c->n || c->max_len <= (u32)DISCO_SHORT_MAX || !two_class_ok(c, c->S, c->n, 1, (u32)c->k + 1)) return DISCO_OK;
    const int Sx = c->S;
    DevBuf<u32> ovf;
    CHK(ensure(c, ovf, c->n_alloc));
    CHK(zero_counter(c, CTR_SHORT_MAX));
    hipLaunchKernelGGL(class_flag_kernel, dim3(flat_grid(c, c->n)), dim3(256), 0, c->stream, c->d_len, c->n, ovf.p, c->d_ctr);
    u64 n_long = 0;
    CHK((scan_exclusive<u32, u32>(c, ovf, c->n, ovf, false, &n_long)));
    CHK(read_counters(c));
    const u32 short_max = (u32)c->h_ctr[CTR_SHORT_MAX];
    if (!two_class_ok(c, Sx, c->n, n_long, short_max)) {
        release(c, ovf);
        return DISCO_OK;
    }
    DevBuf<u64> rows8;
    c->d_ovf = ovf;
    int rca = ensure(c, rows8, (c->n + n_long) * 8);
    if (rca == DISCO_OK) rca = two_class_alloc(c, n_long, Sx, short_max);
    if (rca != DISCO_OK) {
        release(c, rows8);
        free_long_class(c);
        return rca;
    }
    hipLaunchKernelGGL(class_split_kernel, dim3(flat_grid(c, c->n * 8)), dim3(256), 0, c->stream, (const u64 *)c->reads_own, Sx, (const u16 *)c->d_len, (const u32 *)ovf, c->n, c->tailb,
                       rows8.p, c->d_full, c->d_long_ids);
    HIPCHK(c, hipGetLastError());
    HIPCHK(c, hipStreamSynchronize(c->stream));
    release(c, c->reads_own);
    c->reads_own = rows8;
    c->d_reads = c->reads_own;
    c->max_len_all = c->max_len;
    c->max_len = short_max;
    return DISCO_OK;
}

int disco_build_index(disco_ctx *c)
{
    DISCO_TRACE("disco_build_index");
    if (!c) return DISCO_E_ARG;
    if (c->phase < 1) return fail(c, DISCO_E_STATE, "disco_build_index: no reads");
    HIPCHK(c, hipSetDevice(c->device));
    ph_begin(c, DISCO_PH_INDEX);
    if (c->index_counted) {
        c->index_counted = false;
    } else {
        CHK(two_class_convert(c));
        CHK(index_begin(c));
        const DiscoView v = view(c);
        IndexCountPlan pl;
        CHK(index_count_plan(c, v, 0, c->n, &pl));
        CHK(index_count_chunk(c, v, pl, !c->binned_index, c->d_rec, 0, c->n));
        if (c->two_class) CHK(index_count_long(c, v, pl, !c->binned_index, c->d_rec, pl.oslot, 0, c->n_long));
    }
    const bool binned = c->binned_index;
    if (!binned) CHK((scan_exclusive<u32, u32>(c, c->d_bkt, c->T + 1, c->d_bkt, false, nullptr)));
    c->order_ready = false;
    if (c->order_counted && c->order_counted_lo == 0 && c->order_counted_hi == c->n && !c->two_class && !getenv("DISCO_NO_ORDERED_FILL")) {
        const u64 order_buckets = 1ull << c->order_counted_bits;
        CHK(ensure(c, c->d_order_own, c->n));
        ph_end(c, DISCO_PH_INDEX);
        ph_begin(c, DISCO_PH_ORDER);
        CHK((scan_exclusive<u32, u32>(c, c->d_ocnt, order_buckets + 1, c->d_ocnt, false, nullptr)));
        hipLaunchKernelGGL(order_scatter_kernel, dim3(flat_grid(c, c->n)), dim3(256), 0, c->stream, c->d_okey, c->d_oslot, c->d_ocnt, 32u - (u32)c->order_counted_bits, (u64)0, c->n, c->d_len, c->d_order_own);
        ph_end(c, DISCO_PH_ORDER);
        ph_begin(c, DISCO_PH_INDEX2);
        if (binned) CHK(binned_build_index(c));
        else hipLaunchKernelGGL(index_fill_ordered_kernel, dim3(flat_grid(c, c->n)), dim3(256), 0, c->stream, c->n, (const u64 *)c->d_order_own, (const ulonglong2 *)c->d_rec, (const u32 *)c->d_bkt, c->d_ent);
        ph_end(c, DISCO_PH_INDEX2);
        HIPCHK(c, hipGetLastError());
        c->order_ready = true;
        c->phase = 2;
        return DISCO_OK;
    }
    if (binned) CHK(binned_build_index(c));
    else if (c->n) hipLaunchKernelGGL(index_fill_kernel, dim3(flat_grid(c, 2 * c->n)), dim3(256), 0, c->stream, 2 * c->n, c->d_rec, c->d_bkt, c->d_ent);
    HIPCHK(c, hipGetLastError());
    ph_end(c, DISCO_PH_INDEX);
    c->phase = 2;
    return DISCO_OK;
}

int disco_probe(disco_ctx *c)
{
    DISCO_TRACE("disco_probe");
    if (!c) return DISCO_E_ARG;
    if (c->phase < 2) return fail(c, DISCO_E_STATE, "disco_probe: build the index first");
    HIPCHK(c, hipSetDevice(c->device));
    CHK(settle_contained_rows(c));
    CHK(settle_keys(c));
    settle_hits_prealloc(c);
    const u64 nq = c->q_hi - c->q_lo;
    CHK(ensure(c, c->d_best, c->n_alloc));
    CHK(ensure(c, c->d_row_start, c->n));
    CHK(ensure(c, c->d_row_cnt, c->n));
    if (c->n_alloc) hipLaunchKernelGGL(fill_u64_kernel, dim3(flat_grid(c, c->n_alloc)), dim3(256), 0, c->stream, c->d_best, c->n_alloc, DISCO_NOKEY);
    HIPCHK(c, hipMemsetAsync(c->d_row_cnt, 0, std::max<u64>(c->n, 1) * sizeof(u32), c->stream));
    const bool use_runs = c->runs_lpr != 0 && c->d_runs && c->q_lo >= c->runs_lo && c->q_hi <= c->runs_lo + c->runs_n;
    const ProbeKernel range_kernel = probe_pick(c, 0, use_runs);
    const int grid = range_kernel.runs ? wq_grid(c, range_kernel.runs, nq, "DISCO_PROBE_WAVES") : wq_grid(c, range_kernel.plain, nq, "DISCO_PROBE_WAVES");
    auto launch_probe = [&](const ProbeArgs &a, const ProbeKernel &k, int g) {
        if (k.runs) hipLaunchKernelGGL(k.runs, dim3(g), dim3(64), 0, c->stream, a, (const u32 *)c->d_runs, c->runs_by_pos ? ~0ull : c->runs_lo);
        else hipLaunchKernelGGL(k.plain, dim3(g), dim3(64), 0, c->stream, a);
    };
    const u64 chunk_slots = use_runs ? PR_CHUNK : PROBE_CHUNK;
    u64 want_hits = nq * 64 + (u64)grid * chunk_slots + (1u << 16);
    u32 want_slow = use_runs ? (u32)std::min<u64>(nq, nq / 64 + 1024 + (c->two_class ? c->n_long : 0)) : 1u;
    u32 want_big = (u32)std::min<u64>(nq, nq / 64 + 1024);
    for (int attempt = 0; attempt < 8; attempt++) {
        if (want_hits > c->d_hits.cap) {
            release(c, c->d_hits);
            size_t fr = 0, tot = 0;
            HIPCHK(c, hipMemGetInfo(&fr, &tot));
            if (want_hits * 8 > fr) {
                u64 can = fr / 8 / 10 * 9;
                if (can < (u64)grid * chunk_slots * 2) return fail(c, DISCO_E_NOMEM, "disco_probe: not enough HBM for the hit buffer (%llu entries wanted)", (unsigned long long)want_hits);
                want_hits = can;
            }
            CHK(ensure(c, c->d_hits, want_hits));
        }
        if (want_slow > c->d_slow_list.cap) CHK(ensure(c, c->d_slow_list, want_slow));
        CHK(grow_big_lists(c, want_big));
        HIPCHK(c, hipMemsetAsync(c->d_bump, 0, sizeof(u64), c->stream));
        HIPCHK(c, hipMemsetAsync(c->d_n_big, 0, sizeof(u32), c->stream));
        HIPCHK(c, hipMemsetAsync(c->d_n_slow, 0, sizeof(u32), c->stream));
        HIPCHK(c, hipMemsetAsync(c->d_ctr + CTR_KMER_HITS, 0, sizeof(u64) * 4, c->stream));
        CHK(zero_counter(c, CTR_MAX_ROW));
        CHK(zero_counter(c, CTR_ES_BIG));
        CHK(zero_counter(c, CTR_ES_MID));
        c->es_big_counted = c->tr_big_counted = false;
        ProbeArgs a;
        a.v = view(c);
        a.hits = c->d_hits;
        a.row_start = c->d_row_start;
        a.row_cnt = c->d_row_cnt;
        c->h_probe_rare.bump = c->d_bump;
        c->h_probe_rare.hits_cap = c->d_hits.cap;
        c->h_probe_rare.big_list = c->d_big_list;
        c->h_probe_rare.big_cnt = c->d_big_cnt;
        c->h_probe_rare.n_big = c->d_n_big;
        c->h_probe_rare.big_cap = c->d_big_list.cap;
        c->h_probe_rare.slow_cap = c->d_slow_list.cap;
        c->h_probe_rare.slow_list = c->d_slow_list;
        c->h_probe_rare.n_slow = c->d_n_slow;
        c->h_probe_rare.ctr = c->d_ctr;
        CHK(ensure(c, c->d_probe_rare, 1));
        HIPCHK(c, hipMemcpyAsync(c->d_probe_rare, &c->h_probe_rare, sizeof(ProbeRare), hipMemcpyHostToDevice, c->stream));
        a.rare = c->d_probe_rare;
        CHK(ensure(c, c->d_meta_ord, std::max<u64>(nq, 1)));
        a.meta_ord = c->d_meta_ord;
        int order_bits = 16;
        const bool own_order = own_order_wanted(c, nq, &order_bits);
        a.order = nullptr;
        const u64 order_buckets = 1ull << order_bits;
        const bool counted = c->order_counted && c->order_counted_lo == c->q_lo && c->order_counted_hi == c->q_hi && c->order_counted_bits == order_bits;
        c->order_counted = false;
        if (c->loci) {
            c->d_order_used = c->d_order_own;
        } else if (own_order && c->order_ready && counted) {
            c->d_order_used = c->d_order_own;
        } else if (own_order) {
            CHK(ensure(c, c->d_ocnt, order_buckets + 1));
            CHK(ensure(c, c->d_oslot, nq));
            CHK(ensure(c, c->d_order_own, nq));
            const u32 oshift = 32u - (u32)order_bits;
            ph_begin(c, DISCO_PH_ORDER);
            if (!counted) {
                HIPCHK(c, hipMemsetAsync(c->d_ocnt, 0, (order_buckets + 1) * sizeof(u32), c->stream));
                hipLaunchKernelGGL(order_count_kernel, dim3(flat_grid(c, nq)), dim3(256), 0, c->stream, c->d_okey + c->q_lo, nq, oshift, c->d_ocnt, c->d_oslot);
            }
            CHK((scan_exclusive<u32, u32>(c, c->d_ocnt, order_buckets + 1, c->d_ocnt, false, nullptr)));
            hipLaunchKernelGGL(order_scatter_kernel, dim3(flat_grid(c, nq)), dim3(256), 0, c->stream, c->d_okey + c->q_lo, c->d_oslot, c->d_ocnt, oshift, c->q_lo, nq, c->d_len, c->d_order_own);
            ph_end(c, DISCO_PH_ORDER);
            HIPCHK(c, hipGetLastError());
            c->d_order_used = c->d_order_own;
        } else if (c->order_external && nq) {
            CHK(ensure(c, c->d_order_own, nq));
            hipLaunchKernelGGL(order_pack_kernel, dim3(flat_grid(c, nq)), dim3(256), 0, c->stream, c->d_order, nq, c->d_len, c->d_order_own);
            HIPCHK(c, hipGetLastError());
            c->d_order_used = c->d_order_own;
        } else
            c->d_order_used = nullptr;
        a.order = c->d_order_used;
        c->order_q_lo = c->q_lo;
        c->order_q_hi = c->q_hi;
        ph_begin(c, DISCO_PH_PROBE_KERNEL);
        HIPCHK(c, hipMemsetAsync(c->d_wq, 0, sizeof(u64) * WQ_WORDS, c->stream));
        const bool partitioned = c->dist_active && c->part_index;
        if (partitioned) CHK(dist_partitioned_probe(c));
        else if (nq) {
            launch_probe(a, range_kernel, grid);
        }
        ph_end(c, DISCO_PH_PROBE_KERNEL);
        HIPCHK(c, hipGetLastError());
        u32 n_big = 0, n_slow = 0;
        if (!partitioned) {
            HIPCHK(c, hipMemcpyAsync(&n_slow, c->d_n_slow, sizeof(u32), hipMemcpyDeviceToHost, c->stream));
            HIPCHK(c, hipMemcpyAsync(&n_big, c->d_n_big, sizeof(u32), hipMemcpyDeviceToHost, c->stream));
        }
        CHK(read_counters(c));
        if (partitioned) c->h_ctr[CTR_HITS_NEEDED] = c->hits_used;
        if (!c->h_ctr[CTR_OVERFLOW] && n_slow) {
            int g2 = wave_grid(c, (n_slow + WQ_CHUNK - 1) / WQ_CHUNK, 24);
            HIPCHK(c, hipMemsetAsync(c->d_wq, 0, sizeof(u64) * WQ_WORDS, c->stream));
            launch_probe(a, probe_pick(c, 2, false), g2);
            HIPCHK(c, hipGetLastError());
            HIPCHK(c, hipMemcpyAsync(&n_big, c->d_n_big, sizeof(u32), hipMemcpyDeviceToHost, c->stream));
            CHK(read_counters(c));
        }
        if (!partitioned) c->slow_rows = n_slow;
        if (!c->h_ctr[CTR_OVERFLOW] && n_big) {
            int g2 = wave_grid(c, (n_big + WQ_CHUNK - 1) / WQ_CHUNK, 8);
            HIPCHK(c, hipMemsetAsync(c->d_wq, 0, sizeof(u64) * WQ_WORDS, c->stream));
            launch_probe(a, probe_pick(c, 1, false), g2);
            HIPCHK(c, hipGetLastError());
            CHK(read_counters(c));
        }
        if (!c->h_ctr[CTR_OVERFLOW]) {
            c->big_rows = n_big;
            c->hits_used = c->h_ctr[CTR_HITS_NEEDED];
            VerifyArgs va;
            va.v = view(c);
            va.best = c->d_best;
            va.hits = c->d_hits;
            va.row_start = c->d_row_start;
            va.row_cnt = c->d_row_cnt;
            va.order = c->d_order_used;
            va.meta_ord = c->d_meta_ord;
            if (c->wait_bulk_before_verify) {
                HIPCHK(c, hipStreamWaitEvent(c->stream, c->ev_bulk, 0));
                c->wait_bulk_before_verify = false;
            }
            const bool inexact = c->prm.max_substitutions != 0;
            va.max_subs = c->prm.max_substitutions;
            const bool two_pass = !inexact && !c->two_class && (c->prm.flags & DISCO_FLAG_TWO_PASS_VERIFY) && c->S == VERIFY_SW && (nq || c->dist_active) &&
                                  (u64)c->min_len * 10 < (u64)c->max_len * 9 && !getenv("DISCO_NO_TWO_PASS");
            c->two_pass_last = two_pass;
            const bool flat = !inexact && c->S == VERIFY_SW && (c->two_class || !getenv("DISCO_NO_FLAT_VERIFY"));
            ph_begin(c, DISCO_PH_VERIFY);
            if (c->two_class && nq) {
                HIPCHK(c, hipMemsetAsync(c->d_n_list, 0, sizeof(u32), c->stream));
                hipLaunchKernelGGL(class_take_rows_kernel, dim3((unsigned)std::min<u64>((nq + TAKE_SPAN - 1) / TAKE_SPAN, (u64)c->n_cu * 8)), dim3(256), 0, c->stream, c->d_meta_ord,
                                   (const u64 *)c->d_order_used, c->q_lo, nq, (const u32 *)c->d_ovf, c->d_lpos, c->d_lmeta, c->d_linfo, c->d_n_list, (u32)c->n_long);
            }
            if (two_pass) {
                CHK(ensure(c, c->d_contained, c->n_alloc));
                CHK(ensure(c, c->d_cbits, c->n_alloc / 64 + 1));
                va.cbits = c->d_cbits;
                if (nq) verify_launch(c, va, nq, 1, flat, inexact);
                if (c->dist_active) {
                    CHK(dist_mark_contained(c));
                    c->contained_done = true;
                } else {
                    CHK(zero_counter(c, CTR_N_CONTAINED));
                    hipLaunchKernelGGL(contain_flags_kernel, dim3(flat_grid(c, c->n)), dim3(256), 0, c->stream, c->d_best, c->n, c->d_contained, c->d_cbits, c->d_ctr);
                }
                if (nq) verify_launch(c, va, nq, 2, flat, inexact);
            } else if (nq) {
                va.cbits = nullptr;
                verify_launch(c, va, nq, 0, flat, inexact);
            }
            if (c->two_class && nq)
                wq_launch(c, verify_long_kernel, c->n_long * 16, "DISCO_VL_WAVES", 32, va, (const u32 *)c->d_lpos, (const ulonglong2 *)c->d_lmeta, (const uint2 *)c->d_linfo, (const u32 *)c->d_n_list);
            ph_end(c, DISCO_PH_VERIFY);
            HIPCHK(c, hipGetLastError());
            CHK(read_counters(c));
            ph_collect(c);
            c->es_big_counted = true;
            c->phase = 3;
            return DISCO_OK;
        }
        if (getenv("DISCO_VERBOSE"))
            fprintf(stderr, "[disco] probe attempt %d overflowed: hits_cap=%llu needed=%llu n_big=%u big_cap=%u overflow=%llu\n", attempt,
                    (unsigned long long)c->d_hits.cap, (unsigned long long)c->h_ctr[CTR_HITS_NEEDED], n_big, (unsigned)c->d_big_list.cap, (unsigned long long)c->h_ctr[CTR_OVERFLOW]);
        if (n_big > c->d_big_list.cap) want_big = (u32)std::min<u64>(nq, (u64)n_big + n_big / 4 + 1024);
        if (n_slow > c->d_slow_list.cap) want_slow = (u32)std::min<u64>(nq, (u64)n_slow + n_slow / 4 + 1024);
        u64 needed = c->h_ctr[CTR_HITS_NEEDED];
        want_hits = std::max<u64>(c->d_hits.cap * 2, needed + needed / 4 + (u64)grid * chunk_slots);
    }
    return fail(c, DISCO_E_CAPACITY, "disco_probe: hit buffer could not be sized");
}


int disco_mark_contained(disco_ctx *c, uint64_t *n_contained)
{
    DISCO_TRACE("disco_mark_contained");
    if (!c) return DISCO_E_ARG;
    if (c->phase < 3) return fail(c, DISCO_E_STATE, "disco_mark_contained: run disco_probe first");
    HIPCHK(c, hipSetDevice(c->device));
    CHK(ensure(c, c->d_contained, c->n_alloc));
    CHK(ensure(c, c->d_cbits, c->n_alloc / 64 + 1));
    CHK(zero_counter(c, CTR_N_CONTAINED));
    ph_begin(c, DISCO_PH_CONTAIN);
    if (c->n) hipLaunchKernelGGL(contain_flags_kernel, dim3(flat_grid(c, c->n)), dim3(256), 0, c->stream, c->d_best, c->n, c->d_contained, c->d_cbits, c->d_ctr);
    HIPCHK(c, hipGetLastError());
    ph_end(c, DISCO_PH_CONTAIN);
    CHK(read_counters(c));
    ph_collect(c);
    c->n_contained = c->h_ctr[CTR_N_CONTAINED];
    if (n_contained) *n_contained = c->n_contained;
    c->phase = 4;
    c->crows_pending = c->cgrp_pending = false;
    return DISCO_OK;
}

static int ensure_big_cap(disco_ctx *c, const u32 *cnt, const u64 *ref, u32 thr)
{
    CHK(zero_counter(c, CTR_ES_BIG));
// ... 2107 lines not shown
    const u64 total = vsum(adj_totals);
    CHK(ensure(c, deg_all, (u64)G * per));
    CHK(ensure(c, rows_all, std::max<u64>(total, 1)));
    u64 base = 0;
    for (u32 p = 0; p < r; p++) base += adj_totals[p];
    int rc = DISCO_OK;
    const auto t0 = HClock::now();
    do {
        if ((rc = hipMemsetAsync(deg_all + (u64)r * per, 0, per * sizeof(u32), c->stream) == hipSuccess ? DISCO_OK : DISCO_E_HIP) != DISCO_OK) break;
        if ((rc = disco_export_adjacency(c, deg_all + (u64)r * per, rows_all + base)) != DISCO_OK) break;
        if ((rc = c->comm->all_gather(deg_all + (u64)r * per, deg_all, per * sizeof(u32), c->stream)) != DISCO_OK) break;
        std::vector<size_t> off((size_t)G), cnt((size_t)G);
        size_t a = 0;
        for (u32 p = 0; p < G; p++) {
            off[p] = a;
            cnt[p] = adj_totals[p] * sizeof(u64);
            a += cnt[p];
            if (p != r) c->dinfo.bytes_sent[DISCO_X_ADJACENCY] += cnt[r] + per * sizeof(u32);
        }
        if ((rc = c->comm->all_gather_v(rows_all + base, rows_all, off.data(), cnt.data(), c->stream)) != DISCO_OK) break;
        if (hipStreamSynchronize(c->stream) != hipSuccess) {
            rc = DISCO_E_HIP;
            break;
        }
        c->dinfo.ms[DISCO_X_ADJACENCY] += ms_since(t0);
        (void)nloc;
        if ((rc = disco_import_adjacency(c, deg_all, rows_all, total)) != DISCO_OK) break;
        if ((rc = c->comm->all_gather(c->d_dropbits + (u64)r * per / 64, c->d_dropbits, per / 8, c->stream)) != DISCO_OK) break;
        c->dinfo.bytes_sent[DISCO_X_ADJACENCY] += (u64)(G - 1) * (per / 8);
        c->drop_lo = 0;
        c->drop_hi = c->n;
    } while (0);
    release(c, deg_all);
    release(c, rows_all);
    if (rc != DISCO_OK) return c->err.empty() ? fail(c, rc, "adjacency exchange: %s", c->comm->err.c_str()) : rc;
    CHK(disco_symmetrize(c, 1, nullptr));
    CHK(merge_extras(c));
    c->q_lo = 0;
    c->q_hi = c->n;
    rc = disco_transitive_mark(c);
    c->q_lo = lo;
    c->q_hi = hi;
    CHK(rc);
    c->half_complete = true;
    c->dist_active = false;
    c->n_push_r = 0;
    return DISCO_OK;
}

extern "C" {

int disco_comm_unique_id(void *out, size_t cap)
{
    if (!out || cap < DISCO_UNIQUE_ID_BYTES) return DISCO_E_ARG;
    static_assert(sizeof(ncclUniqueId) == DISCO_UNIQUE_ID_BYTES, "unique id size");
    ncclUniqueId id;
    if (ncclGetUniqueId(&id) != ncclSuccess) return fail(nullptr, DISCO_E_HIP, "ncclGetUniqueId failed");
    memcpy(out, &id, sizeof id);
    return DISCO_OK;
}

static int comm_attach(disco_ctx *c, DiscoComm *cm, DiscoComm *bulk)
{
    delete c->comm;
    delete c->comm_bulk;
    c->comm = cm;
    c->comm_bulk = bulk;
    if (hipSetDevice(c->device) != hipSuccess) return fail(c, DISCO_E_HIP, "hipSetDevice failed");
    if (!c->bulk_stream) HIPCHK(c, hipStreamCreateWithFlags(&c->bulk_stream, hipStreamNonBlocking));
    if (!c->ev_bulk) HIPCHK(c, hipEventCreateWithFlags(&c->ev_bulk, hipEventDisableTiming));
    return DISCO_OK;
}

int disco_comm_init(disco_ctx *c, const void *unique_id, int nranks, int rank)
{
    if (!c || !unique_id || nranks < 1 || nranks > DIST_MAX_WORLD || rank < 0 || rank >= nranks) return c ? fail(c, DISCO_E_ARG, "disco_comm_init: bad argument") : DISCO_E_ARG;
    HIPCHK(c, hipSetDevice(c->device));
    const bool one_comm = getenv("DISCO_DIST_ONE_COMM") != nullptr;
    RcclComm *cm = new (std::nothrow) RcclComm();
    RcclComm *bulk = one_comm ? nullptr : new (std::nothrow) RcclComm();
    if (!cm || (!bulk && !one_comm)) {
        delete cm;
        delete bulk;
        return fail(c, DISCO_E_NOMEM, "disco_comm_init: out of host memory");
    }
    int rc = cm->prepare(nranks, rank);
    int bulk_ready = (bulk && bulk->prepare(nranks, rank) == DISCO_OK) ? 1 : 0;
    if (rc == DISCO_OK) rc = cm->join(unique_id);
    if (rc == DISCO_OK && !one_comm) {
        struct IdMsg {
            ncclUniqueId id;
            unsigned long long ok;
        } msg;
        static_assert(sizeof(IdMsg) <= RcclComm::SMALL_VALUES * 8, "fits the staging of host_all_gather");
        memset(&msg, 0, sizeof msg);
        if (rank == 0) msg.ok = ncclGetUniqueId(&msg.id) == ncclSuccess ? 1ull : 0ull;
        void *d_id = cm->d_small;
        memcpy(cm->h_small, &msg, sizeof msg);
        if (hipMemcpyAsync(d_id, cm->h_small, sizeof msg, hipMemcpyHostToDevice, c->stream) != hipSuccess ||
            ncclBroadcast(d_id, d_id, sizeof msg, ncclInt8, 0, cm->comm, c->stream) != ncclSuccess ||
            hipMemcpyAsync(cm->h_small, d_id, sizeof msg, hipMemcpyDeviceToHost, c->stream) != hipSuccess || hipStreamSynchronize(c->stream) != hipSuccess) {
            rc = DISCO_E_HIP;
            cm->err = "broadcast of the second communicator's id failed";
        } else {
            memcpy(&msg, cm->h_small, sizeof msg);
            unsigned long long mine = (msg.ok && bulk_ready) ? 1ull : 0ull, all[DIST_MAX_WORLD];
            rc = cm->host_all_gather(&mine, 1, all, c->stream);
            bool everybody = rc == DISCO_OK;
            for (int p = 0; everybody && p < nranks; p++) everybody = all[p] != 0ull;
            if (rc == DISCO_OK && everybody) {
                const int rb = bulk->join(&msg.id);
                mine = rb == DISCO_OK ? 1ull : 0ull;
                rc = cm->host_all_gather(&mine, 1, all, c->stream);
                for (int p = 0; rc == DISCO_OK && everybody && p < nranks; p++) everybody = all[p] != 0ull;
            }
            if (rc == DISCO_OK && !everybody) {
                if (rank == 0) fprintf(stderr, "[disco] no second communicator on every rank: the reads are gathered on the first one\n");
                delete bulk;
                bulk = nullptr;
            }
        }
    }
    if (one_comm) {
        delete bulk;
        bulk = nullptr;
    }
    if (rc == DISCO_OK && bulk) {
        cm->sibling = bulk;
        bulk->sibling = cm;
    }
    if (rc != DISCO_OK) {
        fail(c, rc, "disco_comm_init: %s %s", cm->err.c_str(), bulk ? bulk->err.c_str() : "");
        delete cm;
        delete bulk;
        return rc;
    }
    return comm_attach(c, cm, bulk);
}

int disco_comm_init_local(disco_ctx *const *ctxs, int nranks)
{
    if (!ctxs || nranks < 1 || nranks > DIST_MAX_WORLD) return DISCO_E_ARG;
    for (int r = 0; r < nranks; r++)
        if (!ctxs[r]) return DISCO_E_ARG;
    auto grp = std::make_shared<LoopGroup>(nranks), grp2 = std::make_shared<LoopGroup>(nranks);
    for (int r = 0; r < nranks; r++) {
        const int rc = comm_attach(ctxs[r], new LoopComm(grp, r), new LoopComm(grp2, r));
        if (rc != DISCO_OK) return rc;
    }
    return DISCO_OK;
}

int disco_probe_run_words(const disco_ctx *c) { return c ? c->runs_lpr : 0; }
int disco_comm_rank(const disco_ctx *c) { return (c && c->comm) ? c->comm->rank : 0; }
int disco_comm_world(const disco_ctx *c) { return (c && c->comm) ? c->comm->world : 1; }
const char *disco_comm_kind(const disco_ctx *c) { return (c && c->comm) ? c->comm->kind() : "none"; }

int disco_dist_range(const disco_ctx *c, uint64_t n_total, uint64_t *lo, uint64_t *hi)
{
    if (!c || !lo || !hi) return DISCO_E_ARG;
    u64 per, l, h;
    dist_range(c, n_total, &per, &l, &h);
    *lo = l;
    *hi = h;
    return DISCO_OK;
}

static int dist_set_reads(disco_ctx *c, u64 n_total, uint32_t dstride)
{
    if (!c->comm) return fail(c, DISCO_E_STATE, "no communicator: call disco_comm_init / disco_comm_init_local first");
    CHK(set_reads_common(c, n_total, dstride));
    u64 per, lo, hi;
    dist_range(c, n_total, &per, &lo, &hi);
    c->per = per;
    c->n_alloc = per * (u64)c->comm->world;
    c->q_lo = c->home_lo = lo;
    c->q_hi = c->home_hi = hi;
    CHK(alloc_reads(c, c->n_alloc * (u64)dstride, c->n_alloc));
    HIPCHK(c, hipMemsetAsync(c->d_reads, 0, c->n_alloc * (u64)dstride * 8, c->stream));
    c->reads_owned = true;
    c->dist_reads = true;
    return DISCO_OK;
}

static int dist_validate(disco_ctx *c)
{
    const u64 nloc = c->q_hi - c->q_lo;
    CHK(zero_counter(c, CTR_BAD_LEN));
    CHK(zero_counter(c, CTR_MAX_LEN));
    CHK(zero_counter(c, CTR_MIN_LEN));
    if (nloc) hipLaunchKernelGGL(validate_len_kernel, dim3(flat_grid(c, nloc)), dim3(256), 0, c->stream, c->d_len + c->q_lo, nloc, c->S, (int)c->prm.min_overlap, c->d_ctr);
    CHK(read_counters(c));
    u64 bad = c->h_ctr[CTR_BAD_LEN], ext[2] = {c->h_ctr[CTR_MAX_LEN], c->h_ctr[CTR_MIN_LEN]};
    CHK(host_reduce(c, &bad, 1));
    CHK(host_reduce(c, ext, 2, true));
    if (bad) return fail(c, DISCO_E_ARG, "%llu reads have a length outside (min_overlap=%u, min(32767, 32*stride)]", (unsigned long long)bad, c->prm.min_overlap);
    c->max_len = (u32)ext[0];
    c->min_len = 0xFFFFu - (u32)ext[1];
    CHK(ensure(c, c->d_list_n, 1));
    HIPCHK(c, hipMemsetAsync(c->d_list_n, 0, sizeof(u64), c->stream));
    if (nloc) hipLaunchKernelGGL(probes_sum_kernel, dim3(flat_grid(c, nloc)), dim3(256), 0, c->stream, c->d_len, c->q_lo, c->q_hi, (u32)c->k, c->d_list_n);
    HIPCHK(c, hipMemcpyAsync(&c->home_probes, c->d_list_n, sizeof(u64), hipMemcpyDeviceToHost, c->stream));
    HIPCHK(c, hipStreamSynchronize(c->stream));
    c->job_n_long = 0;
    c->job_short_max = c->max_len;
    if (c->max_len > (u32)DISCO_SHORT_MAX) {
        DevBuf<u64> d_ls;
        u64 hls[2] = {0, 0};
        CHK(ensure(c, d_ls, 2));
        HIPCHK(c, hipMemsetAsync(d_ls, 0, 2 * sizeof(u64), c->stream));
        if (nloc) hipLaunchKernelGGL(long_stats_kernel, dim3(flat_grid(c, nloc)), dim3(256), 0, c->stream, (const u16 *)c->d_len, c->q_lo, c->q_hi, d_ls);
        HIPCHK(c, hipMemcpyAsync(hls, d_ls, sizeof hls, hipMemcpyDeviceToHost, c->stream));
        HIPCHK(c, hipStreamSynchronize(c->stream));
        release(c, d_ls);
        CHK(host_reduce(c, &hls[0], 1));
        CHK(host_reduce(c, &hls[1], 1, true));
        c->job_n_long = hls[0];
        c->job_short_max = (u32)hls[1];
    }
    c->phase = 1;
    return DISCO_OK;
}

int disco_dist_upload_reads(disco_ctx *c, const uint64_t *packed_own, uint32_t stride_words, const uint16_t *len_own, uint64_t n_total)
{
    DISCO_TRACE("disco_dist_upload_reads");
    if (!c) return DISCO_E_ARG;
    HIPCHK(c, hipSetDevice(c->device));
    const uint32_t dstride = (stride_words + 7u) & ~7u;
    CHK(dist_set_reads(c, n_total, dstride));
    const u64 nloc = c->q_hi - c->q_lo;
    if (nloc && (!packed_own || !len_own)) return fail(c, DISCO_E_ARG, "disco_dist_upload_reads: null argument");
    if (nloc) {
        u64 *dst = c->d_reads + c->q_lo * (u64)dstride;
        if (dstride != stride_words) HIPCHK(c, hipMemsetAsync(dst, 0, nloc * (u64)dstride * 8, c->stream));
        HIPCHK(c, hipMemcpy2DAsync(dst, (size_t)dstride * 8, packed_own, (size_t)stride_words * 8, (size_t)stride_words * 8, nloc, hipMemcpyHostToDevice, c->stream));
        HIPCHK(c, hipMemcpyAsync(c->d_len + c->q_lo, len_own, nloc * 2, hipMemcpyHostToDevice, c->stream));
    }
    return dist_validate(c);
}

int disco_dist_generate_reads(disco_ctx *c, const disco_genspec_abi *s)
{
    DISCO_TRACE("disco_dist_generate_reads");
    if (!c || !s) return c ? fail(c, DISCO_E_ARG, "disco_dist_generate_reads: null argument") : DISCO_E_ARG;
    disco_genspec g;
    memcpy(&g, s, sizeof g);
    const uint32_t longest = std::max<uint32_t>(s->len_max, DISCO_GEN_LONG_SHARE(&g) ? DISCO_GEN_LONG_LEN(&g) : 0u);
    if (s->len_min == 0 || s->len_max < s->len_min || longest > 32767 || s->n_contigs == 0 || s->contig_len < longest)
        return fail(c, DISCO_E_ARG, "disco_dist_generate_reads: bad spec");
    HIPCHK(c, hipSetDevice(c->device));
    const uint32_t stride = (((longest + 31) / 32) + 7u) & ~7u;
    CHK(dist_set_reads(c, s->n_reads, stride));
    const u64 nloc = c->q_hi - c->q_lo;
    if (nloc) hipLaunchKernelGGL(generate_reads_kernel, dim3(flat_grid(c, nloc * stride)), dim3(256), 0, c->stream, g, c->d_reads, c->d_len, (int)stride, c->q_lo, c->q_hi);
    HIPCHK(c, hipGetLastError());
    return dist_validate(c);
}

static int dist_run_graph_pass(disco_ctx *c, uint32_t flags, bool allow_loci, bool *retry_with_id_ranges);

static int dist_run_graph_impl(disco_ctx *c, uint32_t flags)
{
    bool retry = false;
    int rc = dist_run_graph_pass(c, flags, true, &retry);
    if (rc == DISCO_OK && retry) rc = dist_run_graph_pass(c, flags & ~(uint32_t)DISCO_DIST_GATHER_READS, false, &retry);
    return rc;
}

int disco_dist_run_graph(disco_ctx *c, uint32_t flags)
{
    if (c && c->comm)
        c->time_exchanges = getenv("DISCO_DIST_TIME_EXCHANGES") != nullptr ||
                            (c->dist_passes == 0 && c->comm->world > 1 && !strcmp(c->comm->kind(), "rccl") && !getenv("DISCO_DIST_NO_FIRST_CONTACT"));
    const int rc = dist_run_graph_impl(c, flags);
    if (c) c->dist_passes++;
    if (rc != DISCO_OK && c && c->comm && rc != DISCO_E_ARG && rc != DISCO_E_STATE) {
        c->comm->abort();
        if (c->comm_bulk) c->comm_bulk->abort();
    }
    return rc;
}

static int arena_reserve(disco_ctx *c)
{
    if (c->arena.base || getenv("DISCO_DIST_NO_ARENA")) return DISCO_OK;
    const u64 own = c->q_hi - c->q_lo;
    size_t want = (size_t)((double)(own * 760ull + c->n * 46ull) * 1.6) + (256ull << 20);
    if (const char *e = getenv("DISCO_DIST_ARENA_MB")) want = (size_t)atoll(e) << 20;
    size_t fr = 0, tot = 0;
    HIPCHK(c, hipMemGetInfo(&fr, &tot));
    want = std::min(want, fr / 10 * 9);
    void *p = nullptr;
    while (want >= (64ull << 20)) {
        if (hipMalloc(&p, want) == hipSuccess) break;
        (void)hipGetLastError();
        p = nullptr;
        want /= 2;
    }
    if (!p) return DISCO_OK;
    c->arena.base = (char *)p;
    c->arena.size = want & ~(size_t)255;
    c->arena.free_at[0] = c->arena.size;
    return DISCO_OK;
}

// ... 190 lines not shown
```

disco_amd/csrc/disco_kernels.h:

```cpp
#ifndef DISCO_KERNELS_H_
#define DISCO_KERNELS_H_

#include "disco_device.h"
#include "readgen.h"

#define PROBE_ROWCAP 512
#define PROBE_SEGW 128
#define PROBE_SEGP (PROBE_SEGW + 64)
#define PROBE_ACAP 32
#define PROBE_CHUNK 4096
#define ES_MID 1024
#define ES_DUPBITS 11
#define ES_DUPTAB (1 << ES_DUPBITS)
#ifndef ES_CAP
#define ES_CAP 256
#endif
#ifndef TR_CAP
#define TR_CAP 256
#endif
#define TR_CAP_SMALL 128
#define VERIFY_SW 8
#define ORDER_BUCKET(key, shift) (((key) * 0x9E3779B1u) >> (shift))
#define SCAN_ITEMS 16
#define SCAN_BLOCK 256
#define SCAN_TILE (SCAN_ITEMS * SCAN_BLOCK)

#define REF_MAKE(pos, deg) (((u64)(deg) << 40) | (u64)(pos))
#define REF_POS(r) ((r)&0xFFFFFFFFFFull)
#define REF_DEG(r) ((u32)((r) >> 40))
#define ADJ_FLAG (1ull << 15)
#define ADJ_HIDDEN_OF(hit) ((u64)HIT_HIDDEN(hit) << 15)
#define EXTRA_NODE_MAKE(w, slot) ((u64)(w) | ((u64)(slot) << 32))
#define EXTRA_NODE(e) ((e)&0xFFFFFFFFull)
#define EXTRA_SLOT(e) ((u32)((e) >> 32))

enum {
    CTR_KMER_HITS = 0,
    CTR_RAW_HITS,
    CTR_HITS_NEEDED,
    CTR_OVERFLOW,
    CTR_CAP_SITES,
    CTR_ASYM,
    CTR_N_CONTAINED,
    CTR_BAD_LEN,
    CTR_BIG_ROWS,
    CTR_ES_BIG,
    CTR_TR_BIG,
    CTR_MAX_DEG,
    CTR_MAX_ROW,
    CTR_TW_UP,
    CTR_TW_DOWN,
    CTR_ES_SLOW,
    CTR_ADJ_TOTAL,
    CTR_MAX_LEN,
    CTR_DROPPED,
    CTR_MIN_LEN,
    CTR_DROP_ITEMS,
    CTR_SHORT_MAX,
    CTR_TR_MID,
    CTR_ES_MID,
    CTR_COUNT
};

#define WQ_CHUNK 64
#define ORDER_MAKE(id, l) ((u64)(id) | ((u64)(l) << 32))
#define ORDER_ID(o) ((o) & 0xFFFFFFFFull)
#define ORDER_LEN(o) ((int)((o) >> 32))
__device__ __forceinline__ u32 uniform_u32(u32 x) { return (u32)__builtin_amdgcn_readfirstlane((int)x); }
__device__ __forceinline__ u64 uniform_u64(u64 x)
{
    return ((u64)uniform_u32((u32)(x >> 32)) << 32) | uniform_u32((u32)x);
}

template <u32 CHUNK = WQ_CHUNK>
__device__ __forceinline__ bool wq_grab(u64 *counter, u64 n, u64 &beg, u64 &end)
{
    u64 b = 0;
    if ((threadIdx.x & 63) == 0) b = atomicAdd(counter, (u64)CHUNK);
#ifdef WQ_EXP_SHFL
    b = __shfl(b, 0);
#else
    b = uniform_u64(b);
#endif
    beg = b;
    end = (b + CHUNK < n) ? b + CHUNK : n;
    return b < n;
}

template <u32 CHUNK = WQ_CHUNK, u32 MULT = 4>
__device__ __forceinline__ bool wq_grab_multi(u64 *counter, u64 n, u64 &beg, u64 &end, u64 &gnext, u64 &gend)
{
    if (gnext >= gend) {
        if (!wq_grab<CHUNK * MULT>(counter, n, gnext, gend)) return false;
    }
    beg = gnext;
    end = beg + CHUNK < gend ? beg + CHUNK : gend;
    gnext = end;
    return true;
}

#define WQ_NQ 8u
#define WQ_WORDS (16u * WQ_NQ)
struct WqSplit {
    u32 qi = 0;
};
template <u32 CHUNK = WQ_CHUNK>
__device__ __forceinline__ bool wq_grab_split(u64 *counters, u64 n, u64 &beg, u64 &end, WqSplit &st)
{
    const u32 nchunks = (u32)((n + CHUNK - 1u) / CHUNK);
    const u32 per = (nchunks + WQ_NQ - 1u) / WQ_NQ;
    while (st.qi < WQ_NQ) {
        const u32 q = ((u32)blockIdx.x + st.qi) % WQ_NQ;
        const u32 first = q * per;
        const u32 mine = first < nchunks ? (nchunks - first < per ? nchunks - first : per) : 0u;
        u32 b = mine;
        if (mine) {
            u32 t = 0;
            if ((threadIdx.x & 63) == 0) t = atomicAdd((u32 *)&counters[16u * q], 1u);
            b = uniform_u32(t);
        }
        if (b < mine) {
            beg = (u64)(first + b) * CHUNK;
            end = beg + CHUNK < n ? beg + CHUNK : n;
            return true;
        }
        st.qi++;
    }
    return false;
}

struct DiscoView {
    const u64 *reads;
    const u16 *len;
    u64 n;
    int S;
    int k;
    int m;
    const u32 *bkt;
    const u64 *ent;
    int bshift;
    u64 q_lo, q_hi;
    u64 *ctr;
    u64 *wq;
    const u64 *full;
    const u32 *ovf;
    const u32 *long_ids;
    u32 n_long;
    int SL;
    int tailb;
};

struct OwnSet {
    const u8 *otab;
    u32 me;
    u64 lo, hi;
    const u64 *list;
    u64 n_own;
    const u32 *ids;
    __device__ __forceinline__ bool mine(u64 v) const { return otab ? otab[v] == (u8)me : (v >= lo && v < hi); }
    __device__ __forceinline__ u64 count() const { return otab ? n_own : hi - lo; }
    __device__ __forceinline__ u64 node(u64 i) const { return otab ? ORDER_ID(list[i]) : lo + i; }
    __device__ __forceinline__ u64 node_by_id(u64 i) const { return otab ? (u64)ids[i] : lo + i; }
};
__host__ __device__ __forceinline__ u32 disco_key_owner(u32 key, u32 G) { return (u32)(((u64)(key * 0x9E3779B1u) * (u64)G) >> 32); }

__global__ void generate_reads_kernel(disco_genspec spec, u64 *__restrict__ reads, u16 *__restrict__ len, int S, u64 r_lo, u64 r_hi)
{
    u64 gid = r_lo * (u64)S + (u64)blockIdx.x * blockDim.x + threadIdx.x;
    u64 total = r_hi * (u64)S;
    for (; gid < total; gid += (u64)gridDim.x * blockDim.x) {
        u64 r = gid / S;
        int w = (int)(gid % S);
        disco_readloc loc = disco_read_location(&spec, r);
        u64 word = 0;
        int base0 = w * 32;
        for (int i = 0; i < 32; i++) {
            int p = base0 + i;
            if (p < (int)loc.len) word |= (u64)disco_read_base(&spec, &loc, (u32)p) << (62 - 2 * i);
        }
        reads[gid] = word;
        if (w == 0) len[r] = (u16)loc.len;
    }
}

__global__ void substitute_bases_kernel(u64 seed, u32 rate_ppm, u64 *__restrict__ reads, const u16 *__restrict__ len, int S, u64 r_lo, u64 r_hi)
{
    u64 gid = r_lo * (u64)S + (u64)blockIdx.x * blockDim.x + threadIdx.x;
    const u64 total = r_hi * (u64)S;
    for (; gid < total; gid += (u64)gridDim.x * blockDim.x) {
        const u64 r = gid / S;
        const int base0 = (int)(gid % S) * 32, L = (int)len[r];
        if (base0 >= L) continue;
        const u64 word = reads[gid];
        u64 out = 0;
        for (int i = 0; i < 32; i++) {
            u32 b = (u32)(word >> (62 - 2 * i)) & 3u;
            if (base0 + i < L) b = disco_substituted_base(seed, rate_ppm, r, (u32)(base0 + i), b);
            else b = 0;
            out |= (u64)b << (62 - 2 * i);
        }
        reads[gid] = out;
    }
}

__global__ void validate_len_kernel(const u16 *__restrict__ len, u64 n, int S, int min_overlap, u64 *ctr)
{
    u64 i = (u64)blockIdx.x * blockDim.x + threadIdx.x;
    u32 bad = 0, mx = 0, mn = 0xFFFFu;
    for (; i < n; i += (u64)gridDim.x * blockDim.x) {
        u32 L = len[i];
        if (L <= (u32)min_overlap || L > 32767u || L > (u32)S * 32u) bad++;
        mx = L > mx ? L : mx;
        mn = L < mn ? L : mn;
    }
    if (bad) atomicAdd(&ctr[CTR_BAD_LEN], (u64)bad);
    for (int o = 32; o > 0; o >>= 1) {
        mx = max(mx, (u32)__shfl_down(mx, o));
        mn = min(mn, (u32)__shfl_down(mn, o));
    }
    if ((threadIdx.x & 63) == 0) {
        atomicMax(&ctr[CTR_MAX_LEN], (u64)mx);
        atomicMax(&ctr[CTR_MIN_LEN], (u64)(0xFFFFu - mn));
    }
}

template <bool COUNT, bool LONGK = false, bool LONGCLASS = false>
__global__ void __launch_bounds__(256) index_count_kernel(DiscoView v, u32 *__restrict__ bkt, ulonglong2 *__restrict__ rec, u32 *__restrict__ okey, u64 lo, u64 hi,
                                                          u32 *__restrict__ ocnt, u32 *__restrict__ oslot, u32 oshift, const u64 *__restrict__ list = nullptr)
{
    const u64 x = lo + (u64)blockIdx.x * 256u + threadIdx.x;
    if (x >= hi) return;
    const u64 i = LONGCLASS ? (u64)v.long_ids[x] : x;
    const u64 lw = (!LONGCLASS && list) ? list[x] : 0ull;
    const u64 rid = (!LONGCLASS && list) ? ORDER_ID(lw) : i;
    if (LONGCLASS) lo = 0;
    const int S = LONGCLASS ? v.SL : v.S;
    const u64 *__restrict__ p = LONGCLASS ? v.full + x * (u64)S : v.reads + rid * (u64)S;
    if (!LONGCLASS && v.full && v.len[rid] > DISCO_SHORT_MAX) return;
    const int L = (!LONGCLASS && list) ? ORDER_LEN(lw) : (int)v.len[rid], k = v.k, m = v.m, nf = k - m + 1;
    const int nmm = L - m + 1;
    const int sfx0 = nmm - nf;
    const u64 mask = (1ull << (2 * m)) - 1ull;
    const int rsh = 2 * (m - 1);
    u64 f = 0, r = 0, word = 0;
    int pos = 0;
    auto next = [&]() {
        if ((pos & 31) == 0) word = p[pos >> 5];
        const u32 b = (u32)(word >> 62);
        word <<= 2;
        ++pos;
        f = ((f << 2) | b) & mask;
        r = (r >> 2) | ((u64)(3u - b) << rsh);
    };
    u32 best = 0xFFFFFFFFu;
    auto order_word = [&]() {
        next();
        const bool st = r < f;
        const u32 h = order_hash32(st ? r : f);
        best = min(best, h);
        return (h & ~0x1FFu) | (u32)st;
    };
    for (int q = 0; q < m - 1; ++q) next();
    u32 k1p = 0xFFFFFFFFu, k2p = 0xFFFFFFFFu, k1s = 0xFFFFFFFFu, k2s = 0xFFFFFFFFu;
    int q = 0;
    for (; q < nf; ++q) {
        const u32 o = order_word();
        k1p = min(k1p, o + ((u32)q << 1));
        k2p = min(k2p, o + ((u32)(63 - q) << 1));
        if (q >= sfx0) {
            k1s = min(k1s, o + ((u32)(q - sfx0) << 1));
            k2s = min(k2s, o + ((u32)(63 - (q - sfx0)) << 1));
        }
    }
    for (; q < sfx0; ++q) order_word();
    for (; q < nmm; ++q) {
        const u32 o = order_word();
        k1s = min(k1s, o + ((u32)(q - sfx0) << 1));
        k2s = min(k2s, o + ((u32)(63 - (q - sfx0)) << 1));
    }
    if (okey) okey[i] = best;
    if (ocnt) oslot[i - lo] = atomicAdd(&ocnt[ORDER_BUCKET(best, oshift)], 1u);
    auto resolve = [&](u32 k1, u32 k2, int j0, u32 &t, u32 &rev) {
        const int ffirst = (int)((k1 >> 1) & 63u), flast = 63 - (int)((k2 >> 1) & 63u);
        int fsel = ffirst;
        if (ffirst == flast)
            rev = k1 & 1u;
        else {
            rev = kmer_is_rev<false, LONGK>(p, S, j0, k);
            fsel = rev ? flast : ffirst;
        }
        t = rev ? (u32)(nf - 1 - fsel) : (u32)fsel;
        return mmer_key(p, S, j0 + fsel, m);
    };
    u32 tp, rp, ts, rs;
    const u64 kp = resolve(k1p, k2p, 0, tp, rp);
    const u64 ks = resolve(k1s, k2s, sfx0, ts, rs);
    const u64 bp = kp >> v.bshift, bs = ks >> v.bshift;
    const u32 sp = COUNT ? atomicAdd(&bkt[bp], 1u) : 0u;
    const u32 ss = COUNT ? atomicAdd(&bkt[bs], 1u) : 0u;
    rec[2 * (i - lo)] = make_ulonglong2((bp << 32) | sp, PAY_MAKE(kp, rid, tp, rp, 0, L));
    rec[2 * (i - lo) + 1] = make_ulonglong2((bs << 32) | ss, PAY_MAKE(ks, LONGCLASS ? v.n + x : rid, ts, rs, 1, L));
}

#define RUNS_M 23
template <int M>
struct MmerRoll {
    static_assert(M == 0 || (M > 16 && M <= 24 && (M & 1)), "two dwords, the high one partly used; a 24-bit fold in order_hash32<false>");
    const u64 *__restrict__ p;
    int last_word;
    u32 himask, rsh;
    int pos = 0;
    u64 word = 0;
    u32 cw = 0;
    u32 flo = 0, fhi = 0, rlo = 0, rhi = 0;
    bool st = false;
    u32 clo = 0, chi = 0;
    __device__ __forceinline__ MmerRoll(const u64 *row, int S, int m = M) : p(row), last_word(S - 1), himask((1u << (2 * m - 32)) - 1u), rsh((u32)(2 * m - 34)) {}
    __device__ __forceinline__ void step()
    {
        if ((pos & 15) == 0) {
            if ((pos & 31) == 0) word = p[min(pos >> 5, last_word)];
            cw = (pos & 16) ? (u32)word : (u32)(word >> 32);
        }
        const u32 b = __builtin_amdgcn_ubfe(cw, (u32)(30 - 2 * (pos & 15)), 2u);
        ++pos;
        fhi = __builtin_amdgcn_alignbit(fhi, flo, 30u) & (M ? ((1u << (2 * (M ? M : 17) - 32)) - 1u) : himask);
        flo = (flo << 2) | b;
        rlo = __builtin_amdgcn_alignbit(rhi, rlo, 2u);
        rhi = (rhi >> 2) | ((b ^ 3u) << (M ? (u32)(2 * (M ? M : 17) - 34) : rsh));
        st = (((u64)rhi << 32) | rlo) < (((u64)fhi << 32) | flo);
        clo = st ? rlo : flo;
        chi = st ? rhi : fhi;
    }
    __device__ __forceinline__ u32 hash() const { return order_hash32<M == 0>(((u64)chi << 32) | clo); }
    __device__ __forceinline__ u32 strand() const { return st ? 1u : 0u; }
};
#define RUN_W(e) ((u32)(e) >> 7)
#define RUN_DELTA(e) (((u32)(e) >> 1) & 63u)
#define RUN_STRAND(e) ((u32)(e)&1u)
#define OCC_MAKE(slot, e, wend) (((u32)(slot) << 29) | (RUN_STRAND(e) << 23) | (RUN_DELTA(e) << 17) | ((u32)(wend) << 8) | RUN_W(e))
#define OCC_SLOT(d) ((u32)(d) >> 29)
#define OCC_STRAND(d) (((u32)(d) >> 23) & 1u)
#define OCC_DELTA(d) (((u32)(d) >> 17) & 63u)
#define OCC_END(d) (((u32)(d) >> 8) & 0x1FFu)
#define OCC_FIRST(d) ((u32)(d)&0xFFu)

template <bool COUNT, int NF, int NL, int NFMAX = NF, bool LONGK = false>
__global__ void __launch_bounds__(256) index_runs_kernel(DiscoView v, u32 *__restrict__ bkt, ulonglong2 *__restrict__ rec, u32 *__restrict__ okey, u64 lo, u64 hi,
                                                         u32 *__restrict__ runs, u32 *__restrict__ ocnt, u32 *__restrict__ oslot, u32 oshift,
                                                         const u64 *__restrict__ list = nullptr)
{
    static_assert(NF == 0 || NF == NFMAX, "a specialised instantiation holds exactly its window");
    constexpr int CAP = 32 * NL;
    __shared__ u16 s_runs[256 * CAP];
    __shared__ u32 s_x[3 * 256];
    const u32 tid = threadIdx.x;
    for (u32 x = tid; x < 256u * CAP / 2u; x += 256u) ((u32 *)s_runs)[x] = 0xFFFFFFFFu;
    __syncthreads();
    const u64 i = lo + (u64)blockIdx.x * 256u + tid;
    const u64 lw = (list && i < hi) ? list[i] : 0ull;
    const u64 rid = list ? ORDER_ID(lw) : i;
    const bool other_class = i < hi && v.full && v.len[rid] > DISCO_SHORT_MAX;
    if (other_class) s_runs[tid * CAP] = 0xFFFEu;
    if (i < hi && !other_class) {
        const u64 *__restrict__ p = v.reads + rid * v.S;
        const int L = list ? ORDER_LEN(lw) : (int)v.len[rid], k = v.k;
        const int m = NF ? RUNS_M : v.m;
        const int nf = NF ? NF : k - m + 1;
        const int nmm = L - m + 1;
        const int npos = nmm - nf;
        MmerRoll<NF ? RUNS_M : 0> roll(p, v.S, m);
        u32 best = 0xFFFFFFFFu;
        for (int q = 0; q < m - 1; ++q) roll.step();
        u32 s1[NFMAX], s2[NFMAX];
#pragma clang loop unroll(full)
        for (int t = 0; t < NFMAX; ++t) s1[t] = s2[t] = 0xFFFFFFFFu;
        u16 *my = s_runs + tid * CAP;
        u32 cnt = 0, lastm = 0xFFFFFFFFu, tie = 0;
        u32 P1 = 0, P2 = 0;
        u32 *sx = s_x + tid;
        auto window = [&](int w, u32 m1, u32 m2, int base, int tw) {
            if (w <= npos) {
                if (w == npos) {
                    sx[0] = m1;
                    sx[256] = m2;
                    sx[512] = (u32)base;
                } else {
                    tie |= (m1 ^ m2) ^ 0xFEu;
                    if (((m1 ^ lastm) >> 1) != 0u) {
                        lastm = m1;
                        my[cnt < (u32)CAP ? cnt : (u32)CAP - 1u] = (u16)((m1 & 0xFFu) + (((u32)w << 7) - 2u * (u32)tw));
                        ++cnt;
                    }
                }
            }
        };
        const int nblk = npos / nf + 2;
        int q = 0;
        for (int b = 0; b < nblk; ++b) {
            const int base = (b - 1) * nf;
            lastm -= (u32)nf << 1;
            if (b >= 1) window(base, s1[0], s2[0], base, 0);
            if (b == 1) {
                P1 = s1[0];
                P2 = s2[0];
            }
            u32 p1 = 0xFFFFFFFFu, p2 = 0xFFFFFFFFu;
            u32 hc[NFMAX];
#pragma clang loop unroll(full)
            for (int t = 0; t < NFMAX; ++t) {
                if (NF != 0 || t < nf) {
                    roll.step();
                    const u32 h = roll.hash();
                    best = min(best, q < nmm ? h : 0xFFFFFFFFu);
                    const u32 o = (h & ~0x1FFu) | roll.strand();
                    ++q;
                    hc[t] = o;
                    p1 = min(p1, o | ((u32)(nf + t) << 1));
                    p2 = min(p2, o | ((u32)(127 - (nf + t)) << 1));
                    if (t + 1 < nf && b >= 1) window(base + t + 1, min(s1[t + 1 < NFMAX ? t + 1 : 0], p1), min(s2[t + 1 < NFMAX ? t + 1 : 0], p2), base, t + 1);
                }
            }
            u32 a1 = 0xFFFFFFFFu, a2 = 0xFFFFFFFFu;
#pragma clang loop unroll(full)
            for (int t = NFMAX - 1; t >= 0; --t) {
                if (NF == 0 && t >= nf) continue;
                a1 = min(a1, hc[t] | ((u32)t << 1));
                a2 = min(a2, hc[t] | ((u32)(127 - t) << 1));
                s1[t] = a1;
                s2[t] = a2;
            }
        }
        if (okey) okey[i] = best;
        if (ocnt) oslot[i - lo] = atomicAdd(&ocnt[ORDER_BUCKET(best, oshift)], 1u);
        if ((tie & ~1u) != 0 || cnt > (u32)CAP) my[0] = 0xFFFEu;
        auto resolve = [&](u32 k1, u32 k2, int wbase, int j0, u32 &t, u32 &rev) {
            const int ffirst = wbase + (int)((k1 >> 1) & 0x7Fu) - j0, flast = wbase + 127 - (int)((k2 >> 1) & 0x7Fu) - j0;
            int fsel = ffirst;
            if (ffirst == flast)
                rev = k1 & 1u;
            else {
                rev = kmer_is_rev<false, LONGK>(p, v.S, j0, k);
                fsel = rev ? flast : ffirst;
            }
            t = rev ? (u32)(nf - 1 - fsel) : (u32)fsel;
            return mmer_key(p, v.S, j0 + fsel, m);
        };
        u32 tp, rp, ts, rs;
        const u64 kp = resolve(P1, P2, 0, 0, tp, rp);
        const u64 ks = resolve(sx[0], sx[256], (int)sx[512], npos, ts, rs);
        const u64 bp = kp >> v.bshift, bs = ks >> v.bshift;
        const u32 sp = COUNT ? atomicAdd(&bkt[bp], 1u) : 0u;
        const u32 ss = COUNT ? atomicAdd(&bkt[bs], 1u) : 0u;
        rec[2 * (i - lo)] = make_ulonglong2((bp << 32) | sp, PAY_MAKE(kp, rid, tp, rp, 0, L));
        rec[2 * (i - lo) + 1] = make_ulonglong2((bs << 32) | ss, PAY_MAKE(ks, rid, ts, rs, 1, L));
    }
    __syncthreads();
#if defined(INDEX_EXP_NORUNS)
    if (tid != 9999u) return;
#endif
    const u64 r0 = (u64)blockIdx.x * 256u;
    const u64 nr = (hi - lo) - r0 < 256u ? (hi - lo) - r0 : 256u;
    u32 *__restrict__ dst = runs + r0 * (CAP / 2);
    for (u32 x = tid; x < (u32)nr * (CAP / 2); x += 256u) dst[x] = ((const u32 *)s_runs)[x];
}

__global__ void index_fill_kernel(u64 n2, const ulonglong2 *__restrict__ rec, const u32 *__restrict__ bkt, u64 *__restrict__ ent)
{
    u64 i = (u64)blockIdx.x * blockDim.x + threadIdx.x;
    for (; i < n2; i += (u64)gridDim.x * blockDim.x) {
        const ulonglong2 r = rec[i];
        ent[(u64)bkt[r.x >> 32] + (u32)r.x] = r.y;
    }
}

__global__ void index_fill_ordered_kernel(u64 nq, const u64 *__restrict__ order, const ulonglong2 *__restrict__ rec, const u32 *__restrict__ bkt, u64 *__restrict__ ent)
{
    u64 i = (u64)blockIdx.x * blockDim.x + threadIdx.x;
    for (; i < nq; i += (u64)gridDim.x * blockDim.x) {
        const u64 id = ORDER_ID(order[i]);
        const ulonglong2 r0 = rec[2 * id], r1 = rec[2 * id + 1];
        ent[(u64)bkt[r0.x >> 32] + (u32)r0.x] = r0.y;
        ent[(u64)bkt[r1.x >> 32] + (u32)r1.x] = r1.y;
    }
}

#define BINX_SPAN_BITS 14
#define BINX_MAX_BITS 8
#define BINX_TILE 2048u
#define BINX_BLOCK 256u
#define BINX_BUILD_BLOCK 1024u

__device__ __forceinline__ u32 binx_block_scan1024(u32 x, u32 *s_w, u32 *total)
{
    u32 incl = x;
    for (int o = 1; o < 64; o <<= 1) {
        const u32 y = __shfl_up(incl, o);
        if ((int)(threadIdx.x & 63) >= o) incl += y;
    }
    __syncthreads();
    if ((threadIdx.x & 63) == 63) s_w[threadIdx.x >> 6] = incl;
    __syncthreads();
    u32 off = 0, sum = 0;
    for (u32 w = 0; w < 16u; w++) {
        const u32 t = s_w[w];
        off += w < (threadIdx.x >> 6) ? t : 0u;
        sum += t;
    }
    *total = sum;
    return off + incl - x;
}

__global__ void __launch_bounds__(1024) binx_segs_kernel(const u32 *__restrict__ prev_scan, const u32 *__restrict__ ptb, u32 pseg, u32 pnb, u32 total, u32 *__restrict__ seg,
                                                         u32 *__restrict__ tb)
{
    __shared__ u32 s_w[16];
    const u32 nseg = prev_scan ? pseg * pnb : 1u;
    for (u32 x = threadIdx.x; x < nseg; x += 1024u) {
        u32 st = 0;
        if (prev_scan) {
            const u32 s = x / pnb, d = x % pnb;
            const u32 t0 = ptb[s], nt = ptb[s + 1] - t0;
            st = prev_scan[(u64)pnb * t0 + (u64)d * nt];
        }
        seg[x] = st;
    }
    if (threadIdx.x == 0) seg[nseg] = total;
    if (!tb) return;
    __syncthreads();
    u32 carry = 0;
    for (u32 base = 0; base < nseg; base += 1024u) {
        const u32 x = base + threadIdx.x;
        const u32 nt = x < nseg ? (seg[x + 1] - seg[x] + BINX_TILE - 1u) / BINX_TILE : 0u;
        u32 sum;
        const u32 ex = binx_block_scan1024(nt, s_w, &sum);
        if (x < nseg) tb[x] = carry + ex;
        carry += sum;
    }
    if (threadIdx.x == 0) tb[nseg] = carry;
}

__device__ __forceinline__ bool binx_tile(const u32 *__restrict__ seg, const u32 *__restrict__ tb, u32 nseg, u32 &t0, u32 &nt, u32 &ti, u32 &lo, u32 &hi)
{
    const u32 t = blockIdx.x;
    if (t >= tb[nseg]) return false;
    u32 a = 0, b = nseg;
    while (b - a > 1u) {
        const u32 mid = (a + b) >> 1;
        if (tb[mid] <= t) a = mid;
        else b = mid;
    }
    t0 = tb[a];
    nt = tb[a + 1] - t0;
    ti = t - t0;
    const u32 end = seg[a + 1];
    lo = seg[a] + ti * BINX_TILE;
    hi = end - lo > BINX_TILE ? lo + BINX_TILE : end;
    return true;
}

#define BINX_DIGIT(recx, shift, nb) ((u32)((recx) >> (32u + (shift))) & ((nb)-1u))

__global__ void __launch_bounds__(BINX_BLOCK) binx_hist_kernel(const ulonglong2 *__restrict__ rec, const u32 *__restrict__ seg, const u32 *__restrict__ tb, u32 nseg, u32 shift, u32 nb,
                                                               u32 *__restrict__ hist)
{
    __shared__ u32 s_h[1u << BINX_MAX_BITS];
    u32 t0, nt, ti, lo, hi;
    if (!binx_tile(seg, tb, nseg, t0, nt, ti, lo, hi)) return;
    s_h[threadIdx.x] = 0;
    __syncthreads();
    for (u32 i = lo + threadIdx.x; i < hi; i += BINX_BLOCK) atomicAdd(&s_h[BINX_DIGIT(rec[i].x, shift, nb)], 1u);
    __syncthreads();
    if (threadIdx.x < nb) hist[(u64)nb * t0 + (u64)threadIdx.x * nt + ti] = s_h[threadIdx.x];
}

__global__ void __launch_bounds__(BINX_BLOCK) binx_scatter_kernel(const ulonglong2 *__restrict__ src, ulonglong2 *__restrict__ dst, const u32 *__restrict__ seg, const u32 *__restrict__ tb,
                                                                  u32 nseg, u32 shift, u32 nb, const u32 *__restrict__ scan)
{
    static_assert(BINX_BLOCK == (1u << BINX_MAX_BITS) && BINX_TILE % BINX_BLOCK == 0, "a thread per bin; whole rounds per tile");
    constexpr u32 PER = BINX_TILE / BINX_BLOCK;
    __shared__ ulonglong2 s_rec[BINX_TILE];
    __shared__ u32 s_cnt[BINX_BLOCK], s_base[BINX_BLOCK], s_w[BINX_BLOCK / 64u];
    const u32 tid = threadIdx.x;
    u32 t0, nt, ti, lo, hi;
    if (!binx_tile(seg, tb, nseg, t0, nt, ti, lo, hi)) return;
    s_cnt[tid] = 0;
    __syncthreads();
    ulonglong2 r[PER];
    u32 rank[PER];
#pragma unroll
    for (u32 j = 0; j < PER; j++) {
        const u32 i = lo + j * BINX_BLOCK + tid;
        if (i < hi) {
            r[j] = src[i];
            rank[j] = atomicAdd(&s_cnt[BINX_DIGIT(r[j].x, shift, nb)], 1u);
        }
    }
    __syncthreads();
    const u32 cnt = s_cnt[tid];
    u32 incl = cnt;
    for (int o = 1; o < 64; o <<= 1) {
        const u32 y = __shfl_up(incl, o);
        if ((int)(tid & 63u) >= o) incl += y;
    }
    if ((tid & 63u) == 63u) s_w[tid >> 6] = incl;
    __syncthreads();
    u32 start = incl - cnt;
    for (u32 w = 0; w < (tid >> 6); w++) start += s_w[w];
    __syncthreads();
    s_cnt[tid] = start;
    if (tid < nb) s_base[tid] = scan[(u64)nb * t0 + (u64)tid * nt + ti] - start;
    __syncthreads();
#pragma unroll
    for (u32 j = 0; j < PER; j++) {
        const u32 i = lo + j * BINX_BLOCK + tid;
        if (i < hi) s_rec[s_cnt[BINX_DIGIT(r[j].x, shift, nb)] + rank[j]] = r[j];
    }
    __syncthreads();
    for (u32 j = tid; j < hi - lo; j += BINX_BLOCK) {
        const ulonglong2 x = s_rec[j];
        dst[s_base[BINX_DIGIT(x.x, shift, nb)] + j] = x;
    }
}

__global__ void __launch_bounds__(BINX_BUILD_BLOCK) binx_build_kernel(const ulonglong2 *__restrict__ rec, const u32 *__restrict__ part, u32 span, u32 total, u64 T, u32 *__restrict__ bkt,
                                                                      u64 *__restrict__ ent)
{
    __shared__ u32 s_c[1u << BINX_SPAN_BITS];
    __shared__ u32 s_w[16];
    const u32 tid = threadIdx.x, p = blockIdx.x;
    const u32 nbk = 1u << span, mask = nbk - 1u;
    const u32 beg = part[p], end = part[p + 1];
    for (u32 x = tid; x < nbk; x += BINX_BUILD_BLOCK) s_c[x] = 0;
    __syncthreads();
    for (u32 i = beg + tid; i < end; i += BINX_BUILD_BLOCK) atomicAdd(&s_c[(u32)(rec[i].x >> 32) & mask], 1u);
    __syncthreads();
    u32 carry = beg;
    for (u32 base = 0; base < nbk; base += BINX_BUILD_BLOCK) {
        const u32 x = s_c[base + tid];
        u32 sum;
        const u32 ex = binx_block_scan1024(x, s_w, &sum);
        s_c[base + tid] = carry + ex;
        bkt[(u64)p * nbk + base + tid] = carry + ex;
        carry += sum;
    }
    if ((u64)(p + 1u) * nbk == T && tid == 0) bkt[T] = total;
    __syncthreads();
    for (u32 i = beg + tid; i < end; i += BINX_BUILD_BLOCK) {
        const ulonglong2 x = rec[i];
        ent[atomicAdd(&s_c[(u32)(x.x >> 32) & mask], 1u)] = x.y;
    }
}

template <typename InT>
__global__ void __launch_bounds__(SCAN_BLOCK) scan_tile_sums_kernel(const InT *__restrict__ in, u64 n, u64 *__restrict__ tile_sums)
{
    __shared__ u64 s_part[SCAN_BLOCK / DISCO_WAVE];
    u64 base = (u64)blockIdx.x * SCAN_TILE;
    u64 sum = 0;
    for (int i = 0; i < SCAN_ITEMS; i++) {
        u64 idx = base + (u64)i * SCAN_BLOCK + threadIdx.x;
        if (idx < n) sum += (u64)in[idx];
    }
    for (int o = 32; o > 0; o >>= 1) sum += __shfl_down(sum, o);
    if ((threadIdx.x & 63) == 0) s_part[threadIdx.x >> 6] = sum;
    __syncthreads();
    if (threadIdx.x == 0) {
        u64 t = 0;
        for (int w = 0; w < SCAN_BLOCK / DISCO_WAVE; w++) t += s_part[w];
        tile_sums[blockIdx.x] = t;
    }
}

__global__ void __launch_bounds__(1024) scan_sums_kernel(u64 *__restrict__ tile_sums, u64 nt, u64 *__restrict__ total)
{
    __shared__ u64 s_w[16];
    __shared__ u64 s_carry;
    if (threadIdx.x == 0) s_carry = 0;
    __syncthreads();
    for (u64 base = 0; base < nt; base += 1024) {
        u64 idx = base + threadIdx.x;
        u64 x = idx < nt ? tile_sums[idx] : 0;
        u64 incl = x;
        for (int o = 1; o < 64; o <<= 1) {
            u64 y = __shfl_up(incl, o);
            if ((int)(threadIdx.x & 63) >= o) incl += y;
        }
        if ((threadIdx.x & 63) == 63) s_w[threadIdx.x >> 6] = incl;
        __syncthreads();
        u64 woff = 0;
        for (int w = 0; w < (int)(threadIdx.x >> 6); w++) woff += s_w[w];
        u64 carry = s_carry;
        if (idx < nt) tile_sums[idx] = carry + woff + incl - x;
        __syncthreads();
        if (threadIdx.x == 1023) s_carry = carry + woff + incl;
        __syncthreads();
    }
    if (threadIdx.x == 0) *total = s_carry;
}

template <typename InT, typename OutT>
__global__ void __launch_bounds__(SCAN_BLOCK) scan_apply_kernel(const InT *in, u64 n, const u64 *__restrict__ tile_sums, OutT *out)
{
    __shared__ u64 s_w[SCAN_BLOCK / DISCO_WAVE];
    u64 base = (u64)blockIdx.x * SCAN_TILE + (u64)threadIdx.x * SCAN_ITEMS;
    u64 vals[SCAN_ITEMS];
    u64 sum = 0;
#pragma unroll
    for (int i = 0; i < SCAN_ITEMS; i++) {
        u64 idx = base + i;
        vals[i] = idx < n ? (u64)in[idx] : 0;
        sum += vals[i];
    }
    u64 incl = sum;
    for (int o = 1; o < 64; o <<= 1) {
        u64 y = __shfl_up(incl, o);
        if ((int)(threadIdx.x & 63) >= o) incl += y;
    }
    if ((threadIdx.x & 63) == 63) s_w[threadIdx.x >> 6] = incl;
    __syncthreads();
    u64 off = tile_sums[blockIdx.x] + incl - sum;
    for (int w = 0; w < (int)(threadIdx.x >> 6); w++) off += s_w[w];
#pragma unroll
    for (int i = 0; i < SCAN_ITEMS; i++) {
        u64 idx = base + i;
        if (idx < n) out[idx] = (OutT)off;
        off += vals[i];
    }
}

template <typename OutT>
__global__ void scan_write_total_kernel(const u64 *total, OutT *out_n) { *out_n = (OutT)*total; }

struct ProbeRare {
    u64 *bump;
    u64 hits_cap;
    u64 *big_list;
    u32 *big_cnt;
    u32 *n_big;
    u32 big_cap;
    u32 slow_cap;
    u64 *ctr;
    u64 *slow_list;
    u32 *n_slow;
};
struct ProbeArgs {
    DiscoView v;
    u64 *hits;
    u64 *row_start;
    u32 *row_cnt;
    ulonglong2 *meta_ord;
    const ProbeRare *rare;
    const u64 *order;
};

#ifndef PROBE_WAVES_PER_SIMD
#define PROBE_WAVES_PER_SIMD 8
#endif
template <int PMODE, bool LDSROW, bool ROW17, bool LONGK = false, bool LONGCLASS = false>
__global__ void __launch_bounds__(64, (LONGK || LONGCLASS) ? PROBE_WAVES_PER_SIMD - 2 : (ROW17 ? PROBE_WAVES_PER_SIMD - 1 : PROBE_WAVES_PER_SIMD)) probe_kernel(ProbeArgs a)
{
    static_assert(!LONGCLASS || (PMODE != 0 && !LDSROW), "the long class is only ever met in the lists");
    constexpr bool BIG = PMODE == 1, LISTED = PMODE != 0;
    __shared__ u32 s_k1[PROBE_SEGP + 32];
    __shared__ u32 s_k2[PROBE_SEGP + 32];
    __shared__ u8 s_strand[PROBE_SEGP];
    __shared__ u32 s_first[PROBE_SEGP];
    __shared__ u16 s_wp[PROBE_SEGW];
    __shared__ u16 s_lead[PROBE_SEGW];
    __shared__ u32 s_occ_fp[64];
    __shared__ u32 s_occ_start[64];
    __shared__ u32 s_occ_excl[64];
    __shared__ u16 s_occ_prel[64];
    __shared__ u8 s_mark[64];
    __shared__ u64 s_a[PROBE_ACAP + 2];
    const u32 lane = threadIdx.x;
    const int S = a.v.S, k = a.v.k;
    const int m = a.v.m, nf = k - m + 1;
    u64 chunk_base = 0;
    u32 chunk_used = PROBE_CHUNK;
    u32 my_maxrow = 0;
    const u64 n_items = BIG ? (u64)min(*a.rare->n_big, a.rare->big_cap) : (PMODE == 2 ? (u64)min(*a.rare->n_slow, a.rare->slow_cap) : (a.v.q_hi - a.v.q_lo));

    u64 pre_w = 0;
    int pre_len = 0;
    u64 cbeg = 0, cend = 0;
    u64 ord_chunk = 0;
    auto rid = [&](u64 it) { return readlane_u64(ord_chunk, (u32)(it - cbeg)); };
    while (wq_grab(a.v.wq, n_items, cbeg, cend)) {
    if (!LISTED) {
        const u64 i = min(cbeg + lane, cend - 1);
        ord_chunk = a.order ? a.order[i] : ORDER_MAKE(a.v.q_lo + i, a.v.len[a.v.q_lo + i]);
    }
    if (!LISTED && LDSROW) {
        const u64 o0 = rid(cbeg);
        const u64 A0 = ORDER_ID(o0);
        pre_len = ORDER_LEN(o0);
        if ((int)lane < S) pre_w = a.v.reads[A0 * S + lane];
    }
    for (u64 it = cbeg; it < cend; it++) {
        const u64 bl = BIG ? a.rare->big_list[it] : (PMODE == 2 ? a.rare->slow_list[it] : 0ull);
        const u64 oe = LISTED ? 0ull : rid(it);
        const u64 A = LISTED ? (bl & 0xFFFFFFFFull) : ORDER_ID(oe);
// ... 3594 lines not shown
```

Baseline: 10.72 billion overlaps/s.

## Build read order with binned partition sort instead of atomic bucket counting

When the read count is large, the index-count kernel now writes a packed 64-bit item (bucket key, length, read id) per read instead of doing a global atomic increment into order buckets. The order is then built with the existing multi-level binned partition kernels, now templated to handle u64 items as well as 128-bit records. This avoids contended global atomics and a separate scan plus scatter, at the cost of extra partition passes over a reused buffer. The minimizer window loop is also split into an inner range that skips a bounds check, and an inspection API is added to fetch the order.

Result: faster. 10.91 billion overlaps/s (median of 6 runs) (+1.8%).

```diff
diff --git a/disco_amd/build.py b/disco_amd/build.py
--- a/disco_amd/build.py
+++ b/disco_amd/build.py
@@ -11,7 +11,7 @@
 
 HIP_SOURCES = [os.path.join(HERE, "csrc", "disco_hip.hip")]
 HIP_DEPS = HIP_SOURCES + [os.path.join(HERE, "csrc", f) for f in sorted(f for f in os.listdir(os.path.join(HERE, "csrc")) if f.endswith(".h"))] + [
-    os.path.join(ROOT, "include", "disco_hip.h"), os.path.join(ROOT, "include", "disco_hip_test.h")]
+    os.path.join(ROOT, "include", "disco_hip.h"), os.path.join(ROOT, "include", "disco_hip_test.h"), os.path.join(ROOT, "include", "disco_hip_inspect.h")]
 HOST_SOURCES = [os.path.join(HERE, "host", f) for f in ("buildg_main.cpp", "fastx.cpp", "writer.cpp", "parsimple.cpp")]
 
 
diff --git a/disco_amd/buildgraph.py b/disco_amd/buildgraph.py
--- a/disco_amd/buildgraph.py
+++ b/disco_amd/buildgraph.py
@@ -139,6 +139,21 @@
 
 PHASES = ("index", "probe_kernel", "verify", "contain", "select", "csr", "twin", "trmark", "emit", "order")
 
+INSPECT_ABI = [
+    ("disco_fetch_order", C.c_int, [_P, _P, _P, C.c_uint64, C.POINTER(C.c_uint64), C.POINTER(C.c_int)]),
+]
+_inspect_bound = False
+
+
+def _bind_inspect(L):
+    global _inspect_bound
+    if not _inspect_bound:
+        for name, res, args in INSPECT_ABI:
+            fn = getattr(L, name)
+            fn.restype = res
+            fn.argtypes = args
+        _inspect_bound = True
+
 
 def lib_path() -> str:
     return _LIBPATH
@@ -411,6 +426,17 @@
 
     def probe_run_words(self) -> int:
         return int(self.L.disco_probe_run_words(self._h))
+
+    def fetch_order(self):
+        _bind_inspect(self.L)
+        n, bits = C.c_uint64(0), C.c_int(0)
+        one = np.zeros(1, dtype=np.uint64)
+        rc = self.L.disco_fetch_order(self._h, one.ctypes.data, one.ctypes.data, 0, C.byref(n), C.byref(bits))
+        if n.value == 0:
+            self._chk(rc)
+        order, keys = np.zeros(max(n.value, 1), dtype=np.uint64), np.zeros(max(n.value, 1), dtype=np.uint32)
+        self._chk(self.L.disco_fetch_order(self._h, order.ctypes.data, keys.ctypes.data, len(order), C.byref(n), C.byref(bits)))
+        return order[:n.value], keys[:n.value], bits.value
 
     def measure_hbm(self, nbytes: int = 4 << 30, reps: int = 5) -> float:
         out = C.c_double(0.0)
diff --git a/disco_amd/csrc/disco_hip.hip b/disco_amd/csrc/disco_hip.hip
--- a/disco_amd/csrc/disco_hip.hip
+++ b/disco_amd/csrc/disco_hip.hip
@@ -21,6 +21,7 @@
 
 #include "../../include/disco_hip.h"
 #include "../../include/disco_hip_test.h"
+#include "../../include/disco_hip_inspect.h"
 #include "disco_kernels.h"
 #include "disco_dist.h"
 
@@ -208,6 +209,8 @@
     DevBuf<u32> d_ocnt, d_okey, d_oslot;
     DevBuf<u64> d_order_own;
     bool order_counted = false;
+    bool order_items = false;
+    int order_id_bits = 0;
     bool es_big_counted = false, tr_big_counted = false;
     bool contained_count_pending = false;
     bool order_ready = false;
@@ -745,6 +748,7 @@
     const u64 order_min = getenv("DISCO_ORDER_MIN_READS") ? (u64)atoll(getenv("DISCO_ORDER_MIN_READS")) : 4096;
     int b = 16;
     while (b < 27 && (1ull << b) < nq) ++b;
+    if (const char *e = getenv("DISCO_ORDER_BITS")) b = std::min(std::max(atoi(e), 16), 26);
     *bits = b;
     return !c->order_external && !getenv("DISCO_NO_ORDER") && nq >= order_min && nq > 0;
 }
@@ -753,6 +757,8 @@
     u64 lo = 0, hi = 0;
     int lpr = 0, nf = 0;
     u32 *ocnt = nullptr, *oslot = nullptr;
+    u64 *oitem = nullptr;
+    u32 oidbits = 0;
     u32 oshift = 0;
     const u64 *list = nullptr;
 };
@@ -784,6 +790,24 @@
 
 static int two_class_alloc(disco_ctx *c, u64 n_long, int Sx, u32 short_max);
 
+static bool binned_order_wanted(disco_ctx *c, u64 n, int obits, int *id_bits)
+{
+    if (getenv("DISCO_NO_BINNED_ORDER") || getenv("DISCO_NO_ORDERED_FILL") || c->two_class || n != c->n || n >= 0xFFFF0000ull) return false;
+    const u64 binned_min = getenv("DISCO_BINNED_ORDER_MIN_READS") ? (u64)atoll(getenv("DISCO_BINNED_ORDER_MIN_READS")) : (1ull << 21);
+    if (n < binned_min) return false;
+    int idb = 1, lenb = 1;
+    while ((1ull << idb) < n) ++idb;
+    while ((1u << lenb) <= c->max_len) ++lenb;
+    if (obits + lenb + idb > 64) return false;
+    if (ensure(c, c->d_rec2, n) != DISCO_OK) {
+        (void)hipGetLastError();
+        c->err.clear();
+        return false;
+    }
+    *id_bits = idb;
+    return true;
+}
+
 static int index_count_plan(disco_ctx *c, const DiscoView &v, u64 lo, u64 hi, IndexCountPlan *pl, const u64 *list = nullptr)
 {
     const u64 nloc = hi - lo;
@@ -791,15 +815,21 @@
     pl->lo = lo;
     pl->hi = hi;
     pl->list = list;
-    if (!list) c->order_counted = c->order_ready = false;
+    if (!list) c->order_counted = c->order_ready = c->order_items = false;
     int obits = 0;
     if (!list && lo == c->q_lo && hi == c->q_hi && own_order_wanted(c, nloc, &obits) && !getenv("DISCO_NO_ORDER_FUSE")) {
         const u64 order_buckets = 1ull << obits;
-        CHK(ensure(c, c->d_ocnt, order_buckets + 1));
-        CHK(ensure(c, c->d_oslot, nloc));
-        HIPCHK(c, hipMemsetAsync(c->d_ocnt, 0, (order_buckets + 1) * sizeof(u32), c->stream));
-        pl->ocnt = c->d_ocnt;
-        pl->oslot = c->d_oslot;
+        if (lo == 0 && binned_order_wanted(c, nloc, obits, &c->order_id_bits)) {
+            pl->oitem = (u64 *)c->d_rec2.p;
+            pl->oidbits = (u32)c->order_id_bits;
+            c->order_items = true;
+        } else {
+            CHK(ensure(c, c->d_ocnt, order_buckets + 1));
+            CHK(ensure(c, c->d_oslot, nloc));
+            HIPCHK(c, hipMemsetAsync(c->d_ocnt, 0, (order_buckets + 1) * sizeof(u32), c->stream));
+            pl->ocnt = c->d_ocnt;
+            pl->oslot = c->d_oslot;
+        }
         pl->oshift = 32u - (u32)obits;
         c->order_counted = true;
         c->order_counted_lo = lo;
@@ -823,8 +853,8 @@
     return DISCO_OK;
 }
 
-typedef void (*IndexRunsFn)(DiscoView, u32 *, ulonglong2 *, u32 *, u64, u64, u32 *, u32 *, u32 *, u32, const u64 *);
-typedef void (*IndexCountFn)(DiscoView, u32 *, ulonglong2 *, u32 *, u64, u64, u32 *, u32 *, u32, const u64 *);
+typedef void (*IndexRunsFn)(DiscoView, u32 *, ulonglong2 *, u32 *, u64, u64, u32 *, u32 *, u32 *, u64 *, u32, u32, const u64 *);
+typedef void (*IndexCountFn)(DiscoView, u32 *, ulonglong2 *, u32 *, u64, u64, u32 *, u32 *, u64 *, u32, u32, const u64 *);
 struct IndexCountKernel {
     IndexRunsFn runs = nullptr;
     IndexCountFn plain = nullptr;
@@ -872,10 +902,11 @@
     const dim3 grid((unsigned)((b - a + 255) / 256));
     ulonglong2 *rec = rec_base + 2 * (a - pl.lo);
     u32 *oslot = pl.oslot ? pl.oslot + (a - pl.lo) : nullptr;
+    u64 *oitem = pl.oitem ? pl.oitem + (a - pl.lo) : nullptr;
     u32 *okey = pl.list ? nullptr : c->d_okey.p;
     const IndexCountKernel k = index_count_pick(count, pl.nf, v.m, pl.lpr, c->k > 64, false);
-    if (k.runs) hipLaunchKernelGGL(k.runs, grid, dim3(256), 0, c->stream, v, c->d_bkt, rec, okey, a, b, c->d_runs + (a - pl.lo) * (u64)pl.lpr, pl.ocnt, oslot, pl.oshift, pl.list);
-    else hipLaunchKernelGGL(k.plain, grid, dim3(256), 0, c->stream, v, c->d_bkt, rec, okey, a, b, pl.ocnt, oslot, pl.oshift, pl.list);
+    if (k.runs) hipLaunchKernelGGL(k.runs, grid, dim3(256), 0, c->stream, v, c->d_bkt, rec, okey, a, b, c->d_runs + (a - pl.lo) * (u64)pl.lpr, pl.ocnt, oslot, oitem, pl.oidbits, pl.oshift, pl.list);
+    else hipLaunchKernelGGL(k.plain, grid, dim3(256), 0, c->stream, v, c->d_bkt, rec, okey, a, b, pl.ocnt, oslot, oitem, pl.oidbits, pl.oshift, pl.list);
     HIPCHK(c, hipGetLastError());
     return DISCO_OK;
 }
@@ -883,7 +914,7 @@
 static int index_count_long(disco_ctx *c, const DiscoView &v, const IndexCountPlan &pl, bool count, ulonglong2 *rec, u32 *oslot, u64 x_lo, u64 x_hi)
 {
     const dim3 g((unsigned)((x_hi - x_lo + 255) / 256));
-    hipLaunchKernelGGL(index_count_pick(count, 0, v.m, 0, c->k > 64, true).plain, g, dim3(256), 0, c->stream, v, c->d_bkt, rec, c->d_okey, x_lo, x_hi, pl.ocnt, oslot, pl.oshift,
+    hipLaunchKernelGGL(index_count_pick(count, 0, v.m, 0, c->k > 64, true).plain, g, dim3(256), 0, c->stream, v, c->d_bkt, rec, c->d_okey, x_lo, x_hi, pl.ocnt, oslot, (u64 *)nullptr, 0u, pl.oshift,
                        (const u64 *)nullptr);
     HIPCHK(c, hipGetLastError());
     return DISCO_OK;
@@ -942,12 +973,11 @@
     return b;
 }
 
-static int binned_build_index(disco_ctx *c)
-{
-    const int logT = 64 - c->bshift;
-    const BinxPlan bp = binx_plan(logT);
-    const u32 total = (u32)(2 * c->n);
-    const u32 n_part = 1u << (logT - bp.span);
+template <typename R>
+static int binx_partition(disco_ctx *c, const char *what, int bits, u32 kshift, u32 total, R *src, R *dst, const R **out, const u32 **part)
+{
+    const BinxPlan bp = binx_plan(bits);
+    const u32 n_part = 1u << (bits - bp.span);
     const u32 tiles = (total + BINX_TILE - 1u) / BINX_TILE;
     u64 hist_len = 1;
     for (int l = 0, done = 0; l < bp.levels; done += bp.bits[l], l++) hist_len = std::max<u64>(hist_len, ((u64)tiles + (1ull << done)) * (1ull << bp.bits[l]) + 1);
@@ -955,20 +985,18 @@
     CHK(ensure(c, c->d_binx, 4 * tab + hist_len));
     u32 *seg[2] = {c->d_binx.p, c->d_binx.p + tab}, *tb[2] = {c->d_binx.p + 2 * tab, c->d_binx.p + 3 * tab}, *hist = c->d_binx.p + 4 * tab;
     if (getenv("DISCO_VERBOSE"))
-        fprintf(stderr, "[disco] binned index build: 2^%d buckets, %u partitions of 2^%d, %d level(s) of %d / %d / %d bits\n", logT, n_part, bp.span, bp.levels, bp.bits[0], bp.bits[1], bp.bits[2]);
-    ulonglong2 *src = c->d_rec, *dst = c->d_rec2;
+        fprintf(stderr, "[disco] binned %s: 2^%d buckets, %u partitions of 2^%d, %d level(s) of %d / %d / %d bits\n", what, bits, n_part, bp.span, bp.levels, bp.bits[0], bp.bits[1], bp.bits[2]);
     u32 pseg = 1, pnb = 1;
     int cur = 0, done = 0;
     for (int l = 0; l < bp.levels; l++) {
-        const u32 nseg = 1u << done, nb = 1u << bp.bits[l], shift = (u32)(logT - done - bp.bits[l]);
+        const u32 nseg = 1u << done, nb = 1u << bp.bits[l], shift = kshift + (u32)(bits - done - bp.bits[l]);
         const u32 grid = tiles + nseg;
         const u64 hlen = (u64)grid * nb + 1;
         hipLaunchKernelGGL(binx_segs_kernel, dim3(1), dim3(1024), 0, c->stream, l ? (const u32 *)hist : (const u32 *)nullptr, (const u32 *)tb[cur ^ 1], pseg, pnb, total, seg[cur], tb[cur]);
         HIPCHK(c, hipMemsetAsync(hist, 0, hlen * sizeof(u32), c->stream));
-        hipLaunchKernelGGL(binx_hist_kernel, dim3(grid), dim3(BINX_BLOCK), 0, c->stream, (const ulonglong2 *)src, (const u32 *)seg[cur], (const u32 *)tb[cur], nseg, shift, nb, hist);
+        hipLaunchKernelGGL(binx_hist_kernel<R>, dim3(grid), dim3(BINX_BLOCK), 0, c->stream, (const R *)src, (const u32 *)seg[cur], (const u32 *)tb[cur], nseg, shift, nb, hist);
         CHK((scan_exclusive<u32, u32>(c, hist, hlen, hist, false, nullptr)));
-        hipLaunchKernelGGL(binx_scatter_kernel, dim3(grid), dim3(BINX_BLOCK), 0, c->stream, (const ulonglong2 *)src, dst, (const u32 *)seg[cur], (const u32 *)tb[cur], nseg, shift, nb,
-                           (const u32 *)hist);
+        hipLaunchKernelGGL(binx_scatter_kernel<R>, dim3(grid), dim3(BINX_BLOCK), 0, c->stream, (const R *)src, dst, (const u32 *)seg[cur], (const u32 *)tb[cur], nseg, shift, nb, (const u32 *)hist);
         HIPCHK(c, hipGetLastError());
         std::swap(src, dst);
         pseg = nseg;
@@ -978,7 +1006,36 @@
     }
     hipLaunchKernelGGL(binx_segs_kernel, dim3(1), dim3(1024), 0, c->stream, bp.levels ? (const u32 *)hist : (const u32 *)nullptr, (const u32 *)tb[cur ^ 1], pseg, pnb, total, seg[cur],
                        (u32 *)nullptr);
-    hipLaunchKernelGGL(binx_build_kernel, dim3(n_part), dim3(BINX_BUILD_BLOCK), 0, c->stream, (const ulonglong2 *)src, (const u32 *)seg[cur], (u32)bp.span, total, c->T, c->d_bkt.p, c->d_ent.p);
+    HIPCHK(c, hipGetLastError());
+    *out = src;
+    *part = seg[cur];
+    return DISCO_OK;
+}
+
+static int binned_build_index(disco_ctx *c)
+{
+    const int logT = 64 - c->bshift;
+    const u32 total = (u32)(2 * c->n);
+    const ulonglong2 *rec;
+    const u32 *part;
+    CHK(binx_partition(c, "index build", logT, 32u, total, c->d_rec.p, c->d_rec2.p, &rec, &part));
+    const int span = std::min(logT, BINX_SPAN_BITS);
+    hipLaunchKernelGGL(binx_build_kernel<ulonglong2>, dim3(1u << (logT - span)), dim3(BINX_BUILD_BLOCK), 0, c->stream, rec, part, (u32)span, 32u, 0u, total, c->T, c->d_bkt.p, c->d_ent.p);
+    HIPCHK(c, hipGetLastError());
+    return DISCO_OK;
+}
+
+static int binned_build_order(disco_ctx *c)
+{
+    const int bits = c->order_counted_bits;
+    const u32 total = (u32)c->n, kshift = 64u - (u32)bits;
+    u64 *items = (u64 *)c->d_rec2.p;
+    const u64 *rec;
+    const u32 *part;
+    CHK(binx_partition(c, "grouping", bits, kshift, total, items, items + c->n, &rec, &part));
+    const int span = std::min(bits, BINX_SPAN_BITS);
+    hipLaunchKernelGGL(binx_build_kernel<u64>, dim3(1u << (bits - span)), dim3(BINX_BUILD_BLOCK), 0, c->stream, rec, part, (u32)span, kshift, (u32)c->order_id_bits, total, (u64)0,
+                       (u32 *)nullptr, c->d_order_own.p);
     HIPCHK(c, hipGetLastError());
     return DISCO_OK;
 }
@@ -2417,8 +2474,11 @@
         CHK(ensure(c, c->d_order_own, c->n));
         ph_end(c, DISCO_PH_INDEX);
         ph_begin(c, DISCO_PH_ORDER);
-        CHK((scan_exclusive<u32, u32>(c, c->d_ocnt, order_buckets + 1, c->d_ocnt, false, nullptr)));
-        hipLaunchKernelGGL(order_scatter_kernel, dim3(flat_grid(c, c->n)), dim3(256), 0, c->stream, c->d_okey, c->d_oslot, c->d_ocnt, 32u - (u32)c->order_counted_bits, (u64)0, c->n, c->d_len, c->d_order_own);
+        if (c->order_items) CHK(binned_build_order(c));
+        else {
+            CHK((scan_exclusive<u32, u32>(c, c->d_ocnt, order_buckets + 1, c->d_ocnt, false, nullptr)));
+            hipLaunchKernelGGL(order_scatter_kernel, dim3(flat_grid(c, c->n)), dim3(256), 0, c->stream, c->d_okey, c->d_oslot, c->d_ocnt, 32u - (u32)c->order_counted_bits, (u64)0, c->n, c->d_len, c->d_order_own);
+        }
         ph_end(c, DISCO_PH_ORDER);
         ph_begin(c, DISCO_PH_INDEX2);
         if (binned) CHK(binned_build_index(c));
@@ -2509,7 +2569,8 @@
         const bool own_order = own_order_wanted(c, nq, &order_bits);
         a.order = nullptr;
         const u64 order_buckets = 1ull << order_bits;
-        const bool counted = c->order_counted && c->order_counted_lo == c->q_lo && c->order_counted_hi == c->q_hi && c->order_counted_bits == order_bits;
+        const bool counted = c->order_counted && c->order_counted_lo == c->q_lo && c->order_counted_hi == c->q_hi && c->order_counted_bits == order_bits &&
+                             (!c->order_items || c->order_ready);
         c->order_counted = false;
         if (c->loci) {
             c->d_order_used = c->d_order_own;
@@ -4923,6 +4984,20 @@
 }
 
 int disco_probe_run_words(const disco_ctx *c) { return c ? c->runs_lpr : 0; }
+
+int disco_fetch_order(disco_ctx *c, uint64_t *order_words, uint32_t *keys, uint64_t cap, uint64_t *n, int *order_bits)
+{
+    if (!c || !order_words || !keys || !n || !order_bits) return DISCO_E_ARG;
+    if (!c->order_ready || !c->d_order_own || !c->d_okey) return fail(c, DISCO_E_STATE, "disco_fetch_order: disco_build_index made no order");
+    *n = c->n;
+    *order_bits = c->order_counted_bits;
+    if (cap < c->n) return fail(c, DISCO_E_ARG, "disco_fetch_order: room for %llu reads, %llu needed", (unsigned long long)cap, (unsigned long long)c->n);
+    HIPCHK(c, hipSetDevice(c->device));
+    HIPCHK(c, hipMemcpyAsync(order_words, c->d_order_own, c->n * sizeof(u64), hipMemcpyDeviceToHost, c->stream));
+    HIPCHK(c, hipMemcpyAsync(keys, c->d_okey, c->n * sizeof(u32), hipMemcpyDeviceToHost, c->stream));
+    HIPCHK(c, hipStreamSynchronize(c->stream));
+    return DISCO_OK;
+}
 int disco_comm_rank(const disco_ctx *c) { return (c && c->comm) ? c->comm->rank : 0; }
 int disco_comm_world(const disco_ctx *c) { return (c && c->comm) ? c->comm->world : 1; }
 const char *disco_comm_kind(const disco_ctx *c) { return (c && c->comm) ? c->comm->kind() : "none"; }
diff --git a/disco_amd/csrc/disco_kernels.h b/disco_amd/csrc/disco_kernels.h
--- a/disco_amd/csrc/disco_kernels.h
+++ b/disco_amd/csrc/disco_kernels.h
@@ -66,6 +66,7 @@
 #define ORDER_MAKE(id, l) ((u64)(id) | ((u64)(l) << 32))
 #define ORDER_ID(o) ((o) & 0xFFFFFFFFull)
 #define ORDER_LEN(o) ((int)((o) >> 32))
+#define ORDER_ITEM(key, shift, id, l, idbits) (((u64)ORDER_BUCKET(key, shift) << (32u + (shift))) | ((u64)(l) << (idbits)) | (u64)(id))
 __device__ __forceinline__ u32 uniform_u32(u32 x) { return (u32)__builtin_amdgcn_readfirstlane((int)x); }
 __device__ __forceinline__ u64 uniform_u64(u64 x)
 {
@@ -226,7 +227,8 @@
 
 template <bool COUNT, bool LONGK = false, bool LONGCLASS = false>
 __global__ void __launch_bounds__(256) index_count_kernel(DiscoView v, u32 *__restrict__ bkt, ulonglong2 *__restrict__ rec, u32 *__restrict__ okey, u64 lo, u64 hi,
-                                                          u32 *__restrict__ ocnt, u32 *__restrict__ oslot, u32 oshift, const u64 *__restrict__ list = nullptr)
+                                                          u32 *__restrict__ ocnt, u32 *__restrict__ oslot, u64 *__restrict__ oitem, u32 oidbits, u32 oshift,
+                                                          const u64 *__restrict__ list = nullptr)
 {
     const u64 x = lo + (u64)blockIdx.x * 256u + threadIdx.x;
     if (x >= hi) return;
@@ -279,7 +281,8 @@
         k2s = min(k2s, o + ((u32)(63 - (q - sfx0)) << 1));
     }
     if (okey) okey[i] = best;
-    if (ocnt) oslot[i - lo] = atomicAdd(&ocnt[ORDER_BUCKET(best, oshift)], 1u);
+    if (oitem) oitem[i - lo] = ORDER_ITEM(best, oshift, rid, L, oidbits);
+    else if (ocnt) oslot[i - lo] = atomicAdd(&ocnt[ORDER_BUCKET(best, oshift)], 1u);
     auto resolve = [&](u32 k1, u32 k2, int j0, u32 &t, u32 &rev) {
         const int ffirst = (int)((k1 >> 1) & 63u), flast = 63 - (int)((k2 >> 1) & 63u);
         int fsel = ffirst;
@@ -303,6 +306,10 @@
 }
 
 #define RUNS_M 23
+template <bool B>
+struct FlagConst {
+    static constexpr bool value = B;
+};
 template <int M>
 struct MmerRoll {
     static_assert(M == 0 || (M > 16 && M <= 24 && (M & 1)), "two dwords, the high one partly used; a 24-bit fold in order_hash32<false>");
@@ -347,7 +354,8 @@
 
 template <bool COUNT, int NF, int NL, int NFMAX = NF, bool LONGK = false>
 __global__ void __launch_bounds__(256) index_runs_kernel(DiscoView v, u32 *__restrict__ bkt, ulonglong2 *__restrict__ rec, u32 *__restrict__ okey, u64 lo, u64 hi,
-                                                         u32 *__restrict__ runs, u32 *__restrict__ ocnt, u32 *__restrict__ oslot, u32 oshift,
+                                                         u32 *__restrict__ runs, u32 *__restrict__ ocnt, u32 *__restrict__ oslot, u64 *__restrict__ oitem, u32 oidbits,
+                                                         u32 oshift,
                                                          const u64 *__restrict__ list = nullptr)
 {
     static_assert(NF == 0 || NF == NFMAX, "a specialised instantiation holds exactly its window");
@@ -362,9 +370,14 @@
     const u64 rid = list ? ORDER_ID(lw) : i;
     const bool other_class = i < hi && v.full && v.len[rid] > DISCO_SHORT_MAX;
     if (other_class) s_runs[tid * CAP] = 0xFFFEu;
-    if (i < hi && !other_class) {
+    const bool mine = i < hi && !other_class;
+    const int L = mine ? (list ? ORDER_LEN(lw) : (int)v.len[rid]) : 0;
+    int npos_lo = mine ? L - v.k : 0x7FFFFFFF;
+    for (int o = 32; o; o >>= 1) npos_lo = min(npos_lo, __shfl_xor(npos_lo, o));
+    npos_lo = __builtin_amdgcn_readfirstlane(npos_lo);
+    if (mine) {
         const u64 *__restrict__ p = v.reads + rid * v.S;
-        const int L = list ? ORDER_LEN(lw) : (int)v.len[rid], k = v.k;
+        const int k = v.k;
         const int m = NF ? RUNS_M : v.m;
         const int nf = NF ? NF : k - m + 1;
         const int nmm = L - m + 1;
@@ -379,9 +392,9 @@
         u32 cnt = 0, lastm = 0xFFFFFFFFu, tie = 0;
         u32 P1 = 0, P2 = 0;
         u32 *sx = s_x + tid;
-        auto window = [&](int w, u32 m1, u32 m2, int base, int tw) {
-            if (w <= npos) {
-                if (w == npos) {
+        auto window = [&](auto inner, int w, u32 m1, u32 m2, int base, int tw) __attribute__((always_inline)) {
+            if (decltype(inner)::value || w <= npos) {
+                if (!decltype(inner)::value && w == npos) {
                     sx[0] = m1;
                     sx[256] = m2;
                     sx[512] = (u32)base;
@@ -397,10 +410,10 @@
         };
         const int nblk = npos / nf + 2;
         int q = 0;
-        for (int b = 0; b < nblk; ++b) {
+        auto block = [&](auto inner, int b) __attribute__((always_inline)) {
             const int base = (b - 1) * nf;
             lastm -= (u32)nf << 1;
-            if (b >= 1) window(base, s1[0], s2[0], base, 0);
+            if (b >= 1) window(inner, base, s1[0], s2[0], base, 0);
             if (b == 1) {
                 P1 = s1[0];
                 P2 = s2[0];
@@ -412,13 +425,13 @@
                 if (NF != 0 || t < nf) {
                     roll.step();
                     const u32 h = roll.hash();
-                    best = min(best, q < nmm ? h : 0xFFFFFFFFu);
+                    best = min(best, decltype(inner)::value || q < nmm ? h : 0xFFFFFFFFu);
                     const u32 o = (h & ~0x1FFu) | roll.strand();
                     ++q;
                     hc[t] = o;
                     p1 = min(p1, o | ((u32)(nf + t) << 1));
                     p2 = min(p2, o | ((u32)(127 - (nf + t)) << 1));
-                    if (t + 1 < nf && b >= 1) window(base + t + 1, min(s1[t + 1 < NFMAX ? t + 1 : 0], p1), min(s2[t + 1 < NFMAX ? t + 1 : 0], p2), base, t + 1);
+                    if (t + 1 < nf && b >= 1) window(inner, base + t + 1, min(s1[t + 1 < NFMAX ? t + 1 : 0], p1), min(s2[t + 1 < NFMAX ? t + 1 : 0], p2), base, t + 1);
                 }
             }
             u32 a1 = 0xFFFFFFFFu, a2 = 0xFFFFFFFFu;
@@ -430,9 +443,13 @@
                 s1[t] = a1;
                 s2[t] = a2;
             }
-        }
+        };
+        int b = 0;
+        for (const int inner_end = npos_lo / nf; b <= inner_end; ++b) block(FlagConst<true>(), b);
+        for (; b < nblk; ++b) block(FlagConst<false>(), b);
         if (okey) okey[i] = best;
-        if (ocnt) oslot[i - lo] = atomicAdd(&ocnt[ORDER_BUCKET(best, oshift)], 1u);
+        if (oitem) oitem[i - lo] = ORDER_ITEM(best, oshift, rid, L, oidbits);
+        else if (ocnt) oslot[i - lo] = atomicAdd(&ocnt[ORDER_BUCKET(best, oshift)], 1u);
         if ((tie & ~1u) != 0 || cnt > (u32)CAP) my[0] = 0xFFFEu;
         auto resolve = [&](u32 k1, u32 k2, int wbase, int j0, u32 &t, u32 &rev) {
             const int ffirst = wbase + (int)((k1 >> 1) & 0x7Fu) - j0, flast = wbase + 127 - (int)((k2 >> 1) & 0x7Fu) - j0;
@@ -559,9 +576,12 @@
     return true;
 }
 
-#define BINX_DIGIT(recx, shift, nb) ((u32)((recx) >> (32u + (shift))) & ((nb)-1u))
-
-__global__ void __launch_bounds__(BINX_BLOCK) binx_hist_kernel(const ulonglong2 *__restrict__ rec, const u32 *__restrict__ seg, const u32 *__restrict__ tb, u32 nseg, u32 shift, u32 nb,
+__device__ __forceinline__ u64 binx_key(const ulonglong2 &r) { return r.x; }
+__device__ __forceinline__ u64 binx_key(u64 r) { return r; }
+#define BINX_DIGIT(key, shift, nb) ((u32)((key) >> (shift)) & ((nb)-1u))
+
+template <typename R>
+__global__ void __launch_bounds__(BINX_BLOCK) binx_hist_kernel(const R *__restrict__ rec, const u32 *__restrict__ seg, const u32 *__restrict__ tb, u32 nseg, u32 shift, u32 nb,
                                                                u32 *__restrict__ hist)
 {
     __shared__ u32 s_h[1u << BINX_MAX_BITS];
@@ -569,31 +589,32 @@
     if (!binx_tile(seg, tb, nseg, t0, nt, ti, lo, hi)) return;
     s_h[threadIdx.x] = 0;
     __syncthreads();
-    for (u32 i = lo + threadIdx.x; i < hi; i += BINX_BLOCK) atomicAdd(&s_h[BINX_DIGIT(rec[i].x, shift, nb)], 1u);
+    for (u32 i = lo + threadIdx.x; i < hi; i += BINX_BLOCK) atomicAdd(&s_h[BINX_DIGIT(binx_key(rec[i]), shift, nb)], 1u);
     __syncthreads();
     if (threadIdx.x < nb) hist[(u64)nb * t0 + (u64)threadIdx.x * nt + ti] = s_h[threadIdx.x];
 }
 
-__global__ void __launch_bounds__(BINX_BLOCK) binx_scatter_kernel(const ulonglong2 *__restrict__ src, ulonglong2 *__restrict__ dst, const u32 *__restrict__ seg, const u32 *__restrict__ tb,
+template <typename R>
+__global__ void __launch_bounds__(BINX_BLOCK) binx_scatter_kernel(const R *__restrict__ src, R *__restrict__ dst, const u32 *__restrict__ seg, const u32 *__restrict__ tb,
                                                                   u32 nseg, u32 shift, u32 nb, const u32 *__restrict__ scan)
 {
     static_assert(BINX_BLOCK == (1u << BINX_MAX_BITS) && BINX_TILE % BINX_BLOCK == 0, "a thread per bin; whole rounds per tile");
     constexpr u32 PER = BINX_TILE / BINX_BLOCK;
-    __shared__ ulonglong2 s_rec[BINX_TILE];
+    __shared__ R s_rec[BINX_TILE];
     __shared__ u32 s_cnt[BINX_BLOCK], s_base[BINX_BLOCK], s_w[BINX_BLOCK / 64u];
     const u32 tid = threadIdx.x;
     u32 t0, nt, ti, lo, hi;
     if (!binx_tile(seg, tb, nseg, t0, nt, ti, lo, hi)) return;
     s_cnt[tid] = 0;
     __syncthreads();
-    ulonglong2 r[PER];
+    R r[PER];
     u32 rank[PER];
 #pragma unroll
     for (u32 j = 0; j < PER; j++) {
         const u32 i = lo + j * BINX_BLOCK + tid;
         if (i < hi) {
             r[j] = src[i];
-            rank[j] = atomicAdd(&s_cnt[BINX_DIGIT(r[j].x, shift, nb)], 1u);
+            rank[j] = atomicAdd(&s_cnt[BINX_DIGIT(binx_key(r[j]), shift, nb)], 1u);
         }
     }
     __syncthreads();
@@ -614,18 +635,22 @@
 #pragma unroll
     for (u32 j = 0; j < PER; j++) {
         const u32 i = lo + j * BINX_BLOCK + tid;
-        if (i < hi) s_rec[s_cnt[BINX_DIGIT(r[j].x, shift, nb)] + rank[j]] = r[j];
+        if (i < hi) s_rec[s_cnt[BINX_DIGIT(binx_key(r[j]), shift, nb)] + rank[j]] = r[j];
     }
     __syncthreads();
     for (u32 j = tid; j < hi - lo; j += BINX_BLOCK) {
-        const ulonglong2 x = s_rec[j];
-        dst[s_base[BINX_DIGIT(x.x, shift, nb)] + j] = x;
-    }
-}
-
-__global__ void __launch_bounds__(BINX_BUILD_BLOCK) binx_build_kernel(const ulonglong2 *__restrict__ rec, const u32 *__restrict__ part, u32 span, u32 total, u64 T, u32 *__restrict__ bkt,
-                                                                      u64 *__restrict__ ent)
-{
+        const R x = s_rec[j];
+        dst[s_base[BINX_DIGIT(binx_key(x), shift, nb)] + j] = x;
+    }
+}
+
+__device__ __forceinline__ u64 binx_payload(const ulonglong2 &r, u32, u32) { return r.y; }
+__device__ __forceinline__ u64 binx_payload(u64 r, u32 kshift, u32 idbits) { return ORDER_MAKE(r & ((1ull << idbits) - 1ull), (r << (64u - kshift)) >> (64u - kshift + idbits)); }
+template <typename R>
+__global__ void __launch_bounds__(BINX_BUILD_BLOCK) binx_build_kernel(const R *__restrict__ rec, const u32 *__restrict__ part, u32 span, u32 kshift, u32 idbits, u32 total, u64 T,
+                                                                      u32 *__restrict__ bkt, u64 *__restrict__ ent)
+{
+    constexpr bool TABLE = sizeof(R) == sizeof(ulonglong2);
     __shared__ u32 s_c[1u << BINX_SPAN_BITS];
     __shared__ u32 s_w[16];
     const u32 tid = threadIdx.x, p = blockIdx.x;
@@ -633,7 +658,7 @@
     const u32 beg = part[p], end = part[p + 1];
     for (u32 x = tid; x < nbk; x += BINX_BUILD_BLOCK) s_c[x] = 0;
     __syncthreads();
-    for (u32 i = beg + tid; i < end; i += BINX_BUILD_BLOCK) atomicAdd(&s_c[(u32)(rec[i].x >> 32) & mask], 1u);
+    for (u32 i = beg + tid; i < end; i += BINX_BUILD_BLOCK) atomicAdd(&s_c[(u32)(binx_key(rec[i]) >> kshift) & mask], 1u);
     __syncthreads();
     u32 carry = beg;
     for (u32 base = 0; base < nbk; base += BINX_BUILD_BLOCK) {
@@ -641,14 +666,14 @@
         u32 sum;
         const u32 ex = binx_block_scan1024(x, s_w, &sum);
         s_c[base + tid] = carry + ex;
-        bkt[(u64)p * nbk + base + tid] = carry + ex;
+        if (TABLE) bkt[(u64)p * nbk + base + tid] = carry + ex;
         carry += sum;
     }
-    if ((u64)(p + 1u) * nbk == T && tid == 0) bkt[T] = total;
+    if (TABLE && (u64)(p + 1u) * nbk == T && tid == 0) bkt[T] = total;
     __syncthreads();
     for (u32 i = beg + tid; i < end; i += BINX_BUILD_BLOCK) {
-        const ulonglong2 x = rec[i];
-        ent[atomicAdd(&s_c[(u32)(x.x >> 32) & mask], 1u)] = x.y;
+        const R x = rec[i];
+        ent[atomicAdd(&s_c[(u32)(binx_key(x) >> kshift) & mask], 1u)] = binx_payload(x, kshift, idbits);
     }
 }
 
diff --git a/include/disco_hip_inspect.h b/include/disco_hip_inspect.h
--- /dev/null
+++ b/include/disco_hip_inspect.h
@@ -0,0 +1,15 @@
+#ifndef DISCO_HIP_INSPECT_H_
+#define DISCO_HIP_INSPECT_H_
+
+#include "disco_hip.h"
+
+#ifdef __cplusplus
+extern "C" {
+#endif
+
+int disco_fetch_order(disco_ctx *ctx, uint64_t *order_words, uint32_t *keys, uint64_t cap, uint64_t *n, int *order_bits);
+
+#ifdef __cplusplus
+}
+#endif
+#endif
```
